# aelefebv/nellie

Hardware: AMD Instinct MI355X
Metric: Mvoxel/s multiscale Frangi (5 sigma) + Label, float32, frame resident in HBM (higher is better)
Workload: dtype f32; 1 GPU; synthetic 1024x1024x1024 float32 volume (N(100,5) noise + Gaussian tube segments, seed 2345), 0.1 um isotropic, 5-scale Frangi + Label, full hot path per step, frame resident in HBM; voxels=1073741824, labels=265, one_pass_scales=5, fast_div_proven=2, hessian_tile_rows=16

## Files before the change

### include/nellie_amd.h

```cpp
#ifndef NELLIE_AMD_H
#define NELLIE_AMD_H

#include <stddef.h>
#include <stdint.h>

#ifdef __cplusplus
extern "C" {
#endif

#define NL_OK      0
#define NL_EINVAL  1
#define NL_ENODEV  2
#define NL_ENOMEM  3
#define NL_EHIP    4
#define NL_ESTATE  5
#define NL_ECOMM   6

#define NL_U8 0
#define NL_I8 1
#define NL_U16 2
#define NL_I16 3
#define NL_U32 4
#define NL_I32 5
#define NL_F32 6
// ... 4 lines not shown
#define NL_FIELD_GAUSS  0
#define NL_FIELD_FROB   1
#define NL_FIELD_FRANGI 2
#define NL_FIELD_VESSELNESS 3

typedef struct nl_ctx nl_ctx;

const char *nl_version(void);

int nl_device_count(int *count, char *err, size_t errlen);
int nl_device_mem_info(int device, int64_t *free_bytes, int64_t *total_bytes, char *err, size_t errlen);
int nl_device_name(int device, char *name, size_t namelen, char *err, size_t errlen);

int nl_ctx_create(nl_ctx **out, int device,
                  int64_t nz_local, int64_t ny, int64_t nx,
                  int64_t gz0, int64_t gnz, int64_t own_lo, int64_t own_hi,
                  char *err, size_t errlen);
int nl_ctx_destroy(nl_ctx *ctx);
int nl_sync(nl_ctx *ctx, char *err, size_t errlen);
int64_t nl_ctx_bytes(int64_t nz_local, int64_t ny, int64_t nx);


int nl_filter_load(nl_ctx *ctx, const void *host, int dtype, int64_t z0, int64_t z1,
                   char *err, size_t errlen);

int nl_input_load(nl_ctx *ctx, const void *host, int dtype, int64_t z0, int64_t z1,
                  char *err, size_t errlen);
int nl_filter_begin(nl_ctx *ctx, char *err, size_t errlen);

int nl_gauss_step(nl_ctx *ctx,
                  const double *wz, int rz, const double *wy, int ry, const double *wx, int rx,
                  int64_t z0, int64_t z1, char *err, size_t errlen);

int nl_gauss_step_ahead(nl_ctx *ctx, const double *wz, int rz, const double *wy, int ry, const double *wx, int rx,
                        int64_t z0, int64_t z1, char *err, size_t errlen);
int nl_gauss_commit(nl_ctx *ctx, char *err, size_t errlen);

int nl_sample_gather(nl_ctx *ctx, int field, int64_t sz, int64_t sy, int64_t sx,
                     float *out, int64_t cap, int64_t *n, char *err, size_t errlen);

int nl_sample_gather_positive(nl_ctx *ctx, int field, int64_t sz, int64_t sy, int64_t sx,
                              float *out, int64_t cap, int64_t *n, char *err, size_t errlen);
int nl_sample_gather_positive_begin(nl_ctx *ctx, int field, int64_t sz, int64_t sy, int64_t sx, int64_t *n_lattice, char *err, size_t errlen);
int nl_sample_gather_positive_end(nl_ctx *ctx, float *out, int64_t cap, int64_t *n, char *err, size_t errlen);

int nl_sample_minmax(nl_ctx *ctx, int field, int64_t sz, int64_t sy, int64_t sx,
                     float *mn, float *mx, int64_t *npos, char *err, size_t errlen);

int nl_sample_hist(nl_ctx *ctx, int field, int64_t sz, int64_t sy, int64_t sx,
                   const float *edges, int nbins, int64_t *counts, char *err, size_t errlen);

int nl_sample_range_hist(nl_ctx *ctx, int field, int64_t sz, int64_t sy, int64_t sx, int nbins, float *mn, float *mx,
                         int64_t *n_positive, int64_t *counts, float *edges, int *valid, char *err, size_t errlen);
int nl_sample_range_hist2(nl_ctx *ctx, int field_a, int field_b, int64_t sz, int64_t sy, int64_t sx, int nbins, float *mn, float *mx,
                          int64_t *npos, int64_t *counts, float *edges, int *valid, char *err, size_t errlen);

int nl_hist_thresholds(const int64_t *counts, const float *edges, int nbins, double *triangle, double *otsu, int *status,
                       char *err, size_t errlen);
int nl_hist_thresholds_ex(const int64_t *counts, const void *edges, int edges_f64, int nbins, double *triangle, double *otsu,
                          double *otsu_var, int *status, char *err, size_t errlen);
int nl_host_hist_thresholds_f32(const float *values, int64_t n, int nbins, double *triangle, double *otsu, int *status,
                                int64_t *counts_out, float *edges_out, char *err, size_t errlen);

int nl_hessian_stats(nl_ctx *ctx, const double spacing[3],
                     float *max_abs, float *max_frob_sq, int *any_inf, char *err, size_t errlen);

int nl_set_frob_norm(nl_ctx *ctx, float max_abs, float max_finite, char *err, size_t errlen);

int nl_vesselness_step(nl_ctx *ctx, float gamma_sq, float alpha_sq, float beta_sq,
                       int use_thr, float thr, int64_t z0, int64_t z1, int64_t *mask_count,
                       char *err, size_t errlen);

int nl_set_spacing(nl_ctx *ctx, const double spacing[3], char *err, size_t errlen);

int nl_vesselness_spec(nl_ctx *ctx, const double spacing[3], float fsq_lo, float fsq_hi, int64_t z0, int64_t z1,
                       float *max_abs, float *max_frob_sq, int *any_inf, int *overflow, char *err, size_t errlen);

int nl_chain_begin(nl_ctx *ctx, int n_scales, char *err, size_t errlen);
int nl_chain_scale(nl_ctx *ctx, const double spacing[3], int64_t sz, int64_t sy, int64_t sx, double alpha_sq, double beta_sq,
                   double division, double margin, double test_scale, int64_t z0, int64_t z1, char *err, size_t errlen);
int nl_chain_flush(nl_ctx *ctx, char *err, size_t errlen);
int nl_chain_finish(nl_ctx *ctx, int *flags, double *gamma, double *max_abs, double *thr, int64_t *mask_count, char *err, size_t errlen);
int nl_chain_log(nl_ctx *ctx, int k, int which, int64_t *counts, float *edges, float *range, double *scalars, char *err, size_t errlen);

int nl_vesselness_resolve(nl_ctx *ctx, float gamma_sq, float alpha_sq, float beta_sq, int use_thr, float thr,
                          int *hit, int64_t *mask_count, char *err, size_t errlen);

int nl_vesselness_count(nl_ctx *ctx, int64_t *mask_count, char *err, size_t errlen);

int nl_set_ndim(nl_ctx *ctx, int ndim, char *err, size_t errlen);

int nl_log2d_step(nl_ctx *ctx, const double *wy2, const double *wy0, const double *wx2, const double *wx0, int r,
                  float s2, int first, int use_mask, char *err, size_t errlen);

int nl_log2d_finish(nl_ctx *ctx, int64_t *n_positive, char *err, size_t errlen);

int nl_filter_finish(nl_ctx *ctx, int64_t z0, int64_t z1, int64_t *n_positive, char *err, size_t errlen);

int nl_remove_edges(nl_ctx *ctx, int margin, int64_t *n_positive, char *err, size_t errlen);

int nl_mask_volume(nl_ctx *ctx, float thr, char *err, size_t errlen);

int nl_mask_volume_fused(nl_ctx *ctx, float thr, int64_t *n_positive, char *err, size_t errlen);
int nl_tail_enqueue(nl_ctx *ctx, int64_t sz, int64_t sy, int64_t sx, double q, char *err, size_t errlen);
int nl_tail_finish(nl_ctx *ctx, int commit, int64_t *n_samples, float *a, float *b, float *gamma, float *thr, int64_t *n_positive,
                   char *err, size_t errlen);
int nl_mask_volume_dev(nl_ctx *ctx, int64_t sz, int64_t sy, int64_t sx, double q, int64_t *n_samples, float *a, float *b, float *gamma,
                       float *thr, char *err, size_t errlen);
int nl_debug_percentile(nl_ctx *ctx, const float *values, int64_t n, double q, float *thr, float *a, float *b, char *err, size_t errlen);

int nl_filter_store(nl_ctx *ctx, float *host, int64_t z0, int64_t z1, char *err, size_t errlen);

int nl_gauss_store(nl_ctx *ctx, float *host, int64_t z0, int64_t z1, char *err, size_t errlen);


int nl_planes_get(nl_ctx *ctx, int field, int64_t z0, int64_t z1, float *host, char *err, size_t errlen);
int nl_planes_put(nl_ctx *ctx, int field, int64_t z0, int64_t z1, const float *host, char *err, size_t errlen);

int nl_comm_unique_id(char *id128, char *err, size_t errlen);
int nl_comm_init(nl_ctx *ctx, int world, int rank, const char *id128, char *err, size_t errlen);
int nl_comm_loopback_id(char *id128, char *err, size_t errlen);

int nl_halo_exchange(nl_ctx *ctx, int field, int64_t depth, char *err, size_t errlen);
int nl_halo_exchange_at(nl_ctx *ctx, int field, int64_t offset, int64_t depth, int async, char *err, size_t errlen);
int nl_comm_init2(nl_ctx *ctx, int world, int rank, const char *id128, char *err, size_t errlen);

int nl_allreduce(nl_ctx *ctx, void *host_inout, int64_t count, int dtype, int op, char *err, size_t errlen);


int nl_label_load_frangi(nl_ctx *ctx, const float *host, int64_t z0, int64_t z1,
                         char *err, size_t errlen);

int nl_label_intensity_mask(nl_ctx *ctx, const void *host_original, int dtype, double thresh,
                            char *err, size_t errlen);
int nl_label_intensity_mask_planes(nl_ctx *ctx, const void *host_original, int dtype, double thresh, int64_t z0, int64_t z1,
                                   char *err, size_t errlen);
int nl_label_intensity_mask_int(nl_ctx *ctx, const void *host_original, int dtype, int64_t thresh, int64_t z0, int64_t z1,
                                char *err, size_t errlen);

int nl_flat_sample_gather(nl_ctx *ctx, int field, int64_t offset, int64_t step,
                          float *out, int64_t cap, int64_t *n, char *err, size_t errlen);

int nl_flat_sample_gather_positive(nl_ctx *ctx, int field, int64_t offset, int64_t step, float *out, int64_t cap,
                                   int64_t *n, char *err, size_t errlen);

int nl_label_run(nl_ctx *ctx, int has_thr, float thr, int64_t min_area, int fill_holes,
                 int64_t *n_labels, char *err, size_t errlen);

int nl_label_pack(nl_ctx *ctx, int has_thr, float thr, char *err, size_t errlen);
int nl_label_bits_get(nl_ctx *ctx, int64_t row0, int64_t nrows, uint64_t *host, char *err, size_t errlen);
int nl_label_bits_put(nl_ctx *ctx, int64_t row0, int64_t nrows, const uint64_t *host, char *err, size_t errlen);
int nl_label_bits_allgather(nl_ctx *ctx, const int64_t *slab_plane0, char *err, size_t errlen);
int nl_label_run_global(nl_ctx *ctx, int64_t min_area, int fill_holes, int64_t *n_labels, char *err, size_t errlen);

int nl_slab_label_pack(nl_ctx *ctx, int has_thr, float thr, char *err, size_t errlen);
int nl_slab_bits_get(nl_ctx *ctx, int which, int64_t plane, uint64_t *host, char *err, size_t errlen);
int nl_slab_bits_put(nl_ctx *ctx, int which, int64_t plane, const uint64_t *host, char *err, size_t errlen);
int nl_slab_bits_exchange(nl_ctx *ctx, int which, char *err, size_t errlen);
int nl_slab_phase(nl_ctx *ctx, int phase, int gather, int64_t block_ints, int32_t *out, int64_t *need_ints, int64_t *nruns,
                  char *err, size_t errlen);
int nl_slab_patch(nl_ctx *ctx, int64_t n, const int32_t *roots, const int32_t *values, char *err, size_t errlen);
int nl_slab_apply(nl_ctx *ctx, int64_t min_area, char *err, size_t errlen);
int nl_slab_majority(nl_ctx *ctx, char *err, size_t errlen);
int nl_slab_number(nl_ctx *ctx, int64_t n_clear, const int32_t *clear, int64_t n_set, const int32_t *set, int64_t *n_local,
                   int32_t *ids_of_set, char *err, size_t errlen);
int nl_slab_paint(nl_ctx *ctx, int64_t base, int64_t n, const int32_t *roots, const int32_t *labels, char *err, size_t errlen);
// ... 152 lines not shown
```

### nellie_amd/csrc/chain.inc

```
#define NL_CHAIN_BINS 256
#define NL_CHAIN_MAX_SCALES 16

struct ChainHist {
    unsigned long long counts[NL_CHAIN_BINS];
    float edges[NL_CHAIN_BINS + 1];
    float pad_[3];
    unsigned int res[8];
};
static_assert(sizeof(ChainHist) == hist_layout(NL_CHAIN_BINS).bytes && offsetof(ChainHist, edges) == hist_layout(NL_CHAIN_BINS).off_edges &&
              offsetof(ChainHist, res) == hist_layout(NL_CHAIN_BINS).off_res, "ChainHist is hist_layout");

enum {
    NL_CF_GAUSS_HIST = 1, NL_CF_RAW_HIST = 2, NL_CF_TRIANGLE = 4, NL_CF_BRACKET = 8, NL_CF_INF = 16, NL_CF_OVERFLOW = 32,
    NL_CF_NORM_RANGE = 64, NL_CF_MISS = 128, NL_CF_EMPTY = 256, NL_CF_VERIFY = 512
};

struct ChainScale {
    float fsq_lo, fsq_hi;
    float gamma_sq, fsq_min;
    int m_inf, flags;
    float norm[2];
    unsigned int stats[4];
    unsigned long long cnt_walk, cnt_resolve;
    float gamma, max_abs, max_frob, thr, thr_cmp, raw_mn, raw_mx, nmn, nmx;
    int status_gauss, status_raw, status_exact;
    double tri[3], otsu[3];
    ChainHist h_gauss, h_raw, h_exact;
};

__device__ inline int wave_argmax_f64(const double *a, int n) {
    const int lane = threadIdx.x & 63;
    double best = 0.0; int at = 0x7fffffff; int first_nan = 0x7fffffff;
    for (int i = lane; i < n; i += 64) {
        const double v = a[i];
        if (v != v) { if (i < first_nan) first_nan = i; }
        else if (at == 0x7fffffff || v > best) { best = v; at = i; }
    }
#pragma unroll
    for (int o = 32; o > 0; o >>= 1) {
        const int onan = __shfl_xor(first_nan, o, 64);
        first_nan = onan < first_nan ? onan : first_nan;
        const double ob = __shfl_xor(best, o, 64);
        const int oa = __shfl_xor(at, o, 64);
        if (oa != 0x7fffffff && (at == 0x7fffffff || ob > best || (ob == best && oa < at))) { best = ob; at = oa; }
    }
    return first_nan != 0x7fffffff ? first_nan : (at == 0x7fffffff ? 0 : at);
}

__device__ inline void dev_hist_thresholds(const unsigned long long *counts, const float *edges, int nbins, double *scratch,
                                           double *triangle, double *otsu, int *status) {
    const int lane = threadIdx.x & 63;
    double *p = scratch, *pc = scratch + nbins, *w1 = scratch + 2 * nbins, *a1 = scratch + 3 * nbins, *w2 = scratch + 4 * nbins,
           *a2 = scratch + 5 * nbins;
    unsigned long long part = 0;
    for (int i = lane; i < nbins; i += 64) part += counts[i];
    const long long total = (long long)wave_sum_u64(part);
    for (int i = lane; i < nbins; i += 64) {
        const float centre = (edges[i] + edges[i + 1]) / 2.0f;
        const double pi = (double)(long long)counts[i] / (double)total;
        p[i] = pi;
        pc[i] = pi * (double)centre;
    }
    __syncthreads();
    if (nbins == 4 * 64) {
        double pv[4], qv[4], o1[4], o2[4];
#pragma unroll
        for (int j = 0; j < 4; ++j) { pv[j] = p[4 * lane + j]; qv[j] = pc[4 * lane + j]; }
        auto bcast = [](double v, int src) -> double {
            const unsigned long long b = (unsigned long long)__double_as_longlong(v);
            const unsigned int lo = (unsigned int)__builtin_amdgcn_readlane((int)(unsigned int)b, src);
            const unsigned int hi = (unsigned int)__builtin_amdgcn_readlane((int)(unsigned int)(b >> 32), src);
            return __longlong_as_double((long long)(((unsigned long long)hi << 32) | lo));
        };
        double acc = 0.0, accm = 0.0;
        for (int src = 0; src < 64; ++src) {
            double a = acc, m = accm;
            if (lane == src) {
#pragma unroll
                for (int j = 0; j < 4; ++j) { a += pv[j]; m += qv[j]; o1[j] = a; o2[j] = m; }
            }
            acc = bcast(a, src); accm = bcast(m, src);
        }
#pragma unroll
        for (int j = 0; j < 4; ++j) { w1[4 * lane + j] = o1[j]; a1[4 * lane + j] = o2[j]; }
        acc = 0.0; accm = 0.0;
        for (int src = 63; src >= 0; --src) {
            double a = acc, m = accm;
            if (lane == src) {
#pragma unroll
                for (int j = 3; j >= 0; --j) { a += pv[j]; m += qv[j]; o1[j] = a; o2[j] = m; }
            }
            acc = bcast(a, src); accm = bcast(m, src);
        }
#pragma unroll
        for (int j = 0; j < 4; ++j) { w2[4 * lane + j] = o1[j]; a2[4 * lane + j] = o2[j]; }
    } else if (lane == 0) {
        double acc = 0.0, accm = 0.0;
        for (int i = 0; i < nbins; ++i) { acc += p[i]; accm += pc[i]; w1[i] = acc; a1[i] = accm; }
        acc = 0.0; accm = 0.0;
        for (int i = nbins - 1; i >= 0; --i) { acc += p[i]; accm += pc[i]; w2[i] = acc; a2[i] = accm; }
    }
    __syncthreads();
    if (nbins < 2) *otsu = (double)((edges[0] + edges[1]) / 2.0f);
    else {
        double *var = pc;
        for (int i = lane; i + 1 < nbins; i += 64) {
            const double m1 = a1[i] / w1[i], m2 = a2[i + 1] / w2[i + 1];
            const double d = m1 - m2;
            var[i] = (w1[i] * w2[i + 1]) * (d * d);
        }
        __syncthreads();
        const int at = wave_argmax_f64(var, nbins - 1);
        *otsu = (double)((edges[at] + edges[at + 1]) / 2.0f);
    }
    __syncthreads();
    *status = 0;
    int peak = wave_argmax_f64(p, nbins);
    const double height = p[peak];
    int lo = 0x7fffffff, hi = -1;
    for (int i = lane; i < nbins; i += 64)
        if (p[i] != 0.0) { if (i < lo) lo = i; if (i > hi) hi = i; }
#pragma unroll
    for (int o = 32; o > 0; o >>= 1) {
        const int ol = __shfl_xor(lo, o, 64), oh = __shfl_xor(hi, o, 64);
        lo = ol < lo ? ol : lo; hi = oh > hi ? oh : hi;
    }
    if (lo == 0x7fffffff) lo = -1;
    const bool mirrored = (peak - lo) < (hi - peak);
    if (mirrored) { lo = nbins - hi - 1; peak = nbins - peak - 1; }
    const int span = peak - lo;
    if (span <= 0 || lo < 0) { *status = 1; *triangle = 0.0; return; }
    const double norm = sqrt(height * height + (double)((long long)span * (long long)span));
    const double hn = height / norm, sn = (double)span / norm;
    double *dist = w1;
    __syncthreads();
    for (int k = lane; k < span; k += 64) {
        const int bin = mirrored ? nbins - 1 - (k + lo) : k + lo;
        dist[k] = hn * (double)k - sn * p[bin];
    }
    __syncthreads();
    int level = wave_argmax_f64(dist, span) + lo;
    if (mirrored) level = nbins - level - 1;
    *triangle = (double)((edges[level] + edges[level + 1]) / 2.0f);
}

__device__ inline bool dev_finite_f(float x) { return fabsf(x) <= 3.402823466e38f; }

__global__ void __launch_bounds__(64)
chain_thr1_kernel(ChainScale *cs, double division, double margin, double test_scale) {
    __shared__ double scratch[6 * NL_CHAIN_BINS];
    int flags = 0;
    if (blockIdx.x == 0) {
        float gamma = 1.1920929e-07f;
        double tri0 = 0.0, otsu0 = 0.0;
        int st0 = 0;
        const ChainHist &h = cs->h_gauss;
        const unsigned long long cnt = *(const unsigned long long *)(h.res + 2);
        if (cnt == 0ull || h.res[4] != 1u) flags |= NL_CF_GAUSS_HIST;
        else {
            dev_hist_thresholds(h.counts, h.edges, NL_CHAIN_BINS, scratch, &tri0, &otsu0, &st0);
            if (st0) flags |= NL_CF_TRIANGLE;
            const float g = fminf((float)tri0, (float)otsu0);
            if (g > 0.0f) gamma = g;
        }
        const double g64 = (double)gamma;
        const float gamma_sq = (float)(2.0 * (g64 * g64));
        if (threadIdx.x == 0) {
            cs->gamma = gamma; cs->gamma_sq = gamma_sq;
            cs->tri[0] = tri0; cs->otsu[0] = otsu0; cs->status_gauss = st0;
            if (flags) atomicOr(&cs->flags, flags);
        }
        return;
    }
    float lo = __int_as_float(0x7f800000), hi = __int_as_float(0x7f800000);
    double tri1 = 0.0, otsu1 = 0.0;
    int st1 = 0;
    const ChainHist &h = cs->h_raw;
    const float raw_mn = __uint_as_float(h.res[0]), raw_mx = __uint_as_float(h.res[1]);
    const unsigned long long cnt = *(const unsigned long long *)(h.res + 2);
    if (cnt == 0ull || h.res[4] != 1u || !dev_finite_f(raw_mx)) flags |= NL_CF_RAW_HIST;
    else {
        dev_hist_thresholds(h.counts, h.edges, NL_CHAIN_BINS, scratch, &tri1, &otsu1, &st1);
        if (st1) flags |= NL_CF_TRIANGLE;
        const float tf = fminf((float)tri1, (float)otsu1);
        const double t = (double)tf * test_scale / division;
        const float l = (float)(t * t * (1.0 - margin)), u = (float)(t * t * (1.0 + margin));
        if (!(dev_finite_f(l) && dev_finite_f(u) && u > 0.0f) || !(l <= u)) flags |= NL_CF_BRACKET;
        else { lo = l; hi = u; }
    }
    if (threadIdx.x == 0) {
        cs->tri[1] = tri1; cs->otsu[1] = otsu1; cs->status_raw = st1;
        cs->raw_mn = raw_mn; cs->raw_mx = raw_mx;
        cs->fsq_lo = lo; cs->fsq_hi = hi;
        if (flags) atomicOr(&cs->flags, flags);
    }
}

__global__ void __launch_bounds__(64)
chain_post_kernel(ChainScale *cs) {
    if (threadIdx.x != 0) return;
    int flags = 0;
    const float max_abs32 = __uint_as_float(cs->stats[0]), max_fsq32 = __uint_as_float(cs->stats[1]);
    if (cs->stats[2]) flags |= NL_CF_INF;
    if (cs->stats[3]) flags |= NL_CF_OVERFLOW;
    const float max_abs = (max_abs32 <= 0.0f) ? 1.0f : max_abs32;
    cs->max_abs = max_abs;
    cs->max_frob = sqrtf(max_fsq32) / max_abs;
    cs->norm[0] = max_abs; cs->norm[1] = 0.0f;
    const float mn = cs->raw_mn / max_abs, mx = cs->raw_mx / max_abs;
    cs->nmn = mn; cs->nmx = mx;
    unsigned int *res = cs->h_exact.res;
    res[0] = __float_as_uint(mn); res[1] = __float_as_uint(mx); res[2] = 1u; res[3] = 0u; res[4] = 0u;
    if (!(mn > 0.0f && dev_finite_f(mx)) || (cs->flags & NL_CF_RAW_HIST)) { flags |= NL_CF_NORM_RANGE; res[2] = 0u; }
    cs->flags |= flags;
}

__device__ inline float dev_mask_threshold_on_fsq(float max_abs, float thr) {
    auto pred = [&](float x) -> bool { float fr = sqrtf(x); fr = fr / max_abs; return fr > thr; };
    unsigned int lo = 0u, hi = 0x7f7fffffu;
    if (!pred(__uint_as_float(hi))) return __int_as_float(0x7f800000);
    while (lo < hi) {
        const unsigned int mid = lo + (hi - lo) / 2;
        if (pred(__uint_as_float(mid))) hi = mid; else lo = mid + 1;
    }
    return __uint_as_float(lo);
}

__global__ void __launch_bounds__(64)
chain_thr2_kernel(ChainScale *cs, double division) {
    __shared__ double scratch[6 * NL_CHAIN_BINS];
    int flags = 0, st = 0, m_inf = 0;
    double tri = 0.0, otsu = 0.0;
    float thr = 0.0f, thr_cmp = 0.0f, fsq_min = __int_as_float(0x7f800000);
    const ChainHist &h = cs->h_exact;
    if (h.res[4] != 1u || (cs->flags & NL_CF_NORM_RANGE)) flags |= NL_CF_NORM_RANGE;
    else {
        dev_hist_thresholds(h.counts, h.edges, NL_CHAIN_BINS, scratch, &tri, &otsu, &st);
        if (st) flags |= NL_CF_TRIANGLE;
        thr = fminf((float)tri, (float)otsu);
        thr_cmp = (float)((double)thr / division);
        if (!(cs->max_frob > thr_cmp)) flags |= NL_CF_EMPTY;
        fsq_min = dev_mask_threshold_on_fsq(cs->max_abs, thr_cmp);
        m_inf = (0.0f > thr_cmp) ? 1 : 0;
        if (!(fsq_min >= cs->fsq_lo && fsq_min <= cs->fsq_hi)) flags |= NL_CF_MISS;
    }
    if (threadIdx.x == 0) {
        cs->tri[2] = tri; cs->otsu[2] = otsu; cs->status_exact = st;
        cs->thr = thr; cs->thr_cmp = thr_cmp; cs->fsq_min = fsq_min; cs->m_inf = m_inf;
        cs->flags |= flags;
    }
}

__global__ void __launch_bounds__(256)
chain_init_kernel(ChainScale *cs, int n) {
    const size_t words = sizeof(ChainScale) / 4 * (size_t)n;
    unsigned int *w = (unsigned int *)cs;
    for (size_t i = (size_t)blockIdx.x * blockDim.x + threadIdx.x; i < words; i += (size_t)gridDim.x * blockDim.x) w[i] = 0u;
    __syncthreads();
}
__global__ void __launch_bounds__(64)
chain_init2_kernel(ChainScale *cs, int n) {
    const int k = threadIdx.x;
    if (k < n) { cs[k].h_gauss.res[0] = 0xffffffffu; cs[k].h_raw.res[0] = 0xffffffffu; }
}
```

### nellie_amd/csrc/nellie_hip.hip

```cpp
#include "nl_host.h"

#include "hessian.inc"
#include "hessian_pair.inc"
#include "hv_launch.h"
#include "filter2d.inc"
#include "thresholds.inc"
#include "chain.inc"
#include "percentile.inc"


bool gyx_tiled() {
    static int on = -1;
    if (on < 0) { const char *e = getenv("NELLIE_GYX_TILE"); on = (e && !atoi(e)) ? 0 : 1; }
    return on != 0;
}
static unsigned resolve_grid(unsigned blocks) {
    static long cap = -1;
    if (cap < 0) { const char *e = getenv("NELLIE_RESOLVE_GRID"); cap = e ? atol(e) : 8192; }
    return (cap > 0 && (unsigned)cap < blocks) ? (unsigned)cap : blocks;
}
static int hm_ty() {
    static int v = -1;
    if (v < 0) { const char *e = getenv("NELLIE_HM_TY"); v = (e && atoi(e) == 16) ? 16 : 8; }
    return v;
// ... 66 lines not shown
    if (e != hipSuccess) {
        *count = 0;
        return nl_fail(err, errlen, NL_ENODEV, "hipGetDeviceCount: %s", hipGetErrorString(e));
    }
    *count = n;
    return NL_OK;
}

extern "C" int nl_device_mem_info(int device, int64_t *free_bytes, int64_t *total_bytes, char *err, size_t errlen) {
    NL_HIP(hipSetDevice(device));
    size_t f = 0, t = 0;
    NL_HIP(hipMemGetInfo(&f, &t));
    if (free_bytes) *free_bytes = (int64_t)f;
    if (total_bytes) *total_bytes = (int64_t)t;
    return NL_OK;
}

extern "C" int nl_device_name(int device, char *name, size_t namelen, char *err, size_t errlen) {
    hipDeviceProp_t p;
    NL_HIP(hipGetDeviceProperties(&p, device));
    if (name && namelen) snprintf(name, namelen, "%s (%s, %d CUs)", p.name, p.gcnArchName, p.multiProcessorCount);
    return NL_OK;
}

static int64_t vq_padded_plane(int64_t ny, int64_t nx) { return ((nx + HM_TX - 1) / HM_TX) * HM_TX * (((ny + 31) / 32) * 32); }
static int64_t vq_chunks(int64_t nzl, int64_t ny, int64_t nx) {
    static int64_t lim = 0;
    if (!lim) { const char *e = getenv("NELLIE_VQ_CAP"); lim = (e && atoll(e) > 0) ? atoll(e) : ((int64_t)1 << 28); }
    const int64_t per_chunk = vq_padded_plane(ny, nx) * HM_ZCHUNK;
    int64_t chunks = lim / per_chunk;
    const int64_t need = (nzl + HM_ZCHUNK - 1) / HM_ZCHUNK;
    if (chunks > need) chunks = need;
    return chunks < 1 ? 1 : chunks;
}
static int64_t vq_entries(int64_t nzl, int64_t ny, int64_t nx) { return vq_chunks(nzl, ny, nx) * vq_padded_plane(ny, nx) * HM_ZCHUNK; }
static int64_t vq_spec_regions(int64_t nzl, int64_t ny, int64_t nx) {
    return vq_padded_plane(ny, nx) / 64 * ((nzl + HM_ZCHUNK - 1) / HM_ZCHUNK);
}
static int64_t vq_spec_entries(int64_t nzl, int64_t ny, int64_t nx) {
    static int64_t lim = -1;
    if (lim < 0) { const char *e = getenv("NELLIE_SPEC_MAX_GB"); lim = (e ? atoll(e) : 64) << 30; }
    const int64_t ent = vq_spec_regions(nzl, ny, nx) * HM_SPEC_CAP;
    return ent * 32 <= lim ? ent : 0;
}
int64_t vq_alloc_entries(int64_t nzl, int64_t ny, int64_t nx) {
    const int64_t a = vq_entries(nzl, ny, nx), b = vq_spec_entries(nzl, ny, nx);
    return a > b ? a : b;
}
static int64_t vq_alloc_regions(int64_t nzl, int64_t ny, int64_t nx) {
    const int64_t a = vq_entries(nzl, ny, nx) / HM_REGION, b = vq_spec_entries(nzl, ny, nx) ? vq_spec_regions(nzl, ny, nx) : 0;
    return a > b ? a : b;
}

extern "C" int64_t nl_ctx_bytes(int64_t nz_local, int64_t ny, int64_t nx) {
    const int64_t n = nz_local * ny * nx;
    const int64_t qe = vq_alloc_entries(nz_local, ny, nx);
    return n * (4 * 4 + 3) + qe * 32 + vq_alloc_regions(nz_local, ny, nx) * 4 + (1 << 16) + ((n + SCAN_CHUNK - 1) / SCAN_CHUNK + 1) * 4;
}

extern "C" int nl_ctx_destroy(nl_ctx *c) {
    if (!c) return NL_OK;
    hipSetDevice(c->device);
    if (c->stream) hipStreamSynchronize(c->stream);
    for (auto &kv : c->prof) for (auto &r : kv.second) { hipEventDestroy(r.a); hipEventDestroy(r.b); }
    for (auto &r : c->prof_pool) { hipEventDestroy(r.a); hipEventDestroy(r.b); }
    for (int k = 0; k < 4; ++k) if (c->f[k]) hipFree(c->f[k]);
    for (int k = 0; k < 3; ++k) if (c->m[k]) hipFree(c->m[k]);
    if (c->d_small) hipFree(c->d_small);
    if (c->d_input && !c->input_borrowed) hipFree(c->d_input);
    for (int k = 0; k < 2; ++k) { if (c->d_in_slot[k]) hipFree(c->d_in_slot[k]); if (c->ev_in[k]) hipEventDestroy(c->ev_in[k]); }
    if (c->d_stage_fr) hipFree(c->d_stage_fr);
    if (c->d_stage_lab) hipFree(c->d_stage_lab);
    if (c->ev_staged) hipEventDestroy(c->ev_staged);
    if (c->ev_fetched) hipEventDestroy(c->ev_fetched);
    if (c->side) { hipStreamSynchronize(c->side); hipStreamDestroy(c->side); }
    if (c->ev_side) hipEventDestroy(c->ev_side);
    if (c->ev_main) hipEventDestroy(c->ev_main);
    if (c->ev_ahead) hipEventDestroy(c->ev_ahead);
    if (c->copy_in) hipStreamDestroy(c->copy_in);
    if (c->copy_out) hipStreamDestroy(c->copy_out);
    if (c->d_blk) hipFree(c->d_blk);
    for (int k = 0; k < 4; ++k) if (c->d_2d[k]) hipFree(c->d_2d[k]);
    if (c->d_fsq_cache) hipFree(c->d_fsq_cache);
    if (c->d_vq) hipFree(c->d_vq);
    if (c->mk_scratch) hipFree(c->mk_scratch);
    if (c->mk_act) hipFree(c->mk_act);
    if (c->d_vq_count) hipFree(c->d_vq_count);
    if (c->d_rows) hipFree(c->d_rows);
    if (c->d_ag) hipFree(c->d_ag);
    if (c->d_sl) hipFree(c->d_sl);
    if (c->d_seg_done) hipFree(c->d_seg_done);
    nw_release(c);
    if (c->d_pct) hipFree(c->d_pct);
    if (c->h_pct) hipHostFree(c->h_pct);
    if (c->h_sl) hipHostFree(c->h_sl);
    if (c->d_pack) hipFree(c->d_pack);
    if (c->h_ag) hipHostFree(c->h_ag);
    if (c->gbits[0]) hipFree(c->gbits[0]);
    if (c->gbits[1]) hipFree(c->gbits[1]);
    if (c->grows) hipFree(c->grows);
    if (c->h_small) hipHostFree(c->h_small);
    if (c->h_prefix) hipHostFree(c->h_prefix);
    if (c->t0) hipEventDestroy(c->t0);
    if (c->t1) hipEventDestroy(c->t1);
    if (c->xstream) { hipStreamSynchronize(c->xstream); hipStreamDestroy(c->xstream); }
    if (c->ev_x_main) hipEventDestroy(c->ev_x_main);
    if (c->ev_x_done) hipEventDestroy(c->ev_x_done);
    if (c->d_chain) hipFree(c->d_chain);
    if (c->h_chain) hipHostFree(c->h_chain);
    if (c->ev_chain) hipEventDestroy(c->ev_chain);
    comm_release(c, c->comm2, 2);
    comm_release(c, c->comm, 1);
    if (c->stream) hipStreamDestroy(c->stream);
    delete c;
    return NL_OK;
}

extern "C" int nl_ctx_create(nl_ctx **out, int device, int64_t nzl, int64_t ny, int64_t nx,
                             int64_t gz0, int64_t gnz, int64_t own_lo, int64_t own_hi, char *err, size_t errlen) {
    if (!out) return nl_fail(err, errlen, NL_EINVAL, "out is NULL");
    *out = nullptr;
    if (nzl < 1 || ny < 1 || nx < 1) return nl_fail(err, errlen, NL_EINVAL, "empty volume (%lld,%lld,%lld)", (i64)nzl, (i64)ny, (i64)nx);
    if (gz0 < 0 || gz0 + nzl > gnz) return nl_fail(err, errlen, NL_EINVAL, "slab [%lld,%lld) outside the global volume of %lld planes", (i64)gz0, (i64)(gz0 + nzl), (i64)gnz);
    if (own_lo < 0 || own_hi > nzl || own_lo >= own_hi) return nl_fail(err, errlen, NL_EINVAL, "bad owned range [%lld,%lld)", (i64)own_lo, (i64)own_hi);
    const i64 n = (i64)nzl * ny * nx;
    if (n >= ((i64)1 << 31)) return nl_fail(err, errlen, NL_EINVAL, "local slab of %lld voxels exceeds the int32 label index range; shard over Z", n);
    if (ny > 65535 || nzl > 65535) return nl_fail(err, errlen, NL_EINVAL, "Y and local Z extents must be <= 65535");
    int ndev = 0;
    hipError_t e = hipGetDeviceCount(&ndev);
    if (e != hipSuccess || ndev <= 0)
        return nl_fail(err, errlen, NL_ENODEV, "GPU backend requested but no HIP device is available (%s)", e == hipSuccess ? "0 devices" : hipGetErrorString(e));
    if (device < 0 || device >= ndev) return nl_fail(err, errlen, NL_ENODEV, "GPU backend requested but device %d does not exist (%d devices)", device, ndev);
    NL_HIP(hipSetDevice(device));
    nl_ctx *c = new nl_ctx();
    c->device = device; c->nzl = nzl; c->ny = ny; c->nx = nx; c->gz0 = gz0; c->gnz = gnz;
    c->own_lo = own_lo; c->own_hi = own_hi; c->n = n;
    int rc = NL_OK;
    auto alloc = [&](void **p, size_t bytes) -> bool {
        hipError_t ee = hipMalloc(p, bytes);
        if (ee != hipSuccess) {
            rc = nl_fail(err, errlen, ee == hipErrorOutOfMemory ? NL_ENOMEM : NL_EHIP,
                         "hipMalloc(%zu bytes): %s%s", bytes, hipGetErrorString(ee), ee == hipErrorOutOfMemory ? " [out of memory]" : "");
            return false;
        }
        return true;
    };
    bool ok = true;
    for (int k = 0; k < 4 && ok; ++k) ok = alloc((void **)&c->f[k], (size_t)n * 4);
    const size_t mask_words = (size_t)NL_MASK_SLOTS * nzl * ny * ((nx + 63) / 64);
    const size_t plane_words_bytes = (size_t)nzl * ny * ((nx + 63) / 64) * 8;
    for (int k = 0; k < 3 && ok; ++k) {
        size_t bytes = (size_t)n;
        if (k == 0 && mask_words * 8 > bytes) bytes = mask_words * 8;
        if (plane_words_bytes > bytes) bytes = plane_words_bytes;
        ok = alloc((void **)&c->m[k], bytes);
    }
    if (ok) ok = alloc((void **)&c->d_rows, ((size_t)nzl * ny + 2) * 2 * 4);
    if (ok) ok = alloc(&c->d_small, 1 << 16);
    c->vq_chunks = (int)vq_chunks(nzl, ny, nx);
    {
        const size_t qe = (size_t)vq_alloc_entries(nzl, ny, nx);
        if (ok) ok = alloc((void **)&c->d_vq, qe * 32);
        if (ok) ok = alloc((void **)&c->d_vq_count, (size_t)vq_alloc_regions(nzl, ny, nx) * 4);
        c->spec_ok = vq_spec_entries(nzl, ny, nx) > 0;
    }
    c->blk_cap = (n + SCAN_CHUNK - 1) / SCAN_CHUNK + 1;
    if (ok) ok = alloc(&c->d_blk, (size_t)c->blk_cap * 4);
    if (ok && hipHostMalloc(&c->h_small, 1 << 16, hipHostMallocDefault) != hipSuccess) {
        rc = nl_fail(err, errlen, NL_ENOMEM, "hipHostMalloc failed [out of memory]"); ok = false;
    }
    int side_prio = -1;
    { const char *e = getenv("NELLIE_SIDE_PRIO"); if (e) side_prio = atoi(e); }
    int prio_lo = 0, prio_hi = 0;
    (void)hipDeviceGetStreamPriorityRange(&prio_lo, &prio_hi);
    const int side_p = side_prio < 0 ? prio_hi : (side_prio > 0 ? prio_lo : (prio_lo + prio_hi) / 2);
    if (ok && (hipStreamCreateWithPriority(&c->side, hipStreamNonBlocking, side_p) != hipSuccess ||
               hipEventCreateWithFlags(&c->ev_side, hipEventDisableTiming) != hipSuccess ||
               hipEventCreateWithFlags(&c->ev_main, hipEventDisableTiming) != hipSuccess ||
               hipEventCreateWithFlags(&c->ev_ahead, hipEventDisableTiming) != hipSuccess)) {
        rc = nl_fail(err, errlen, NL_EHIP, "stream/event creation failed"); ok = false;
    }
    if (ok && (hipStreamCreateWithFlags(&c->stream, hipStreamNonBlocking) != hipSuccess ||
               hipEventCreate(&c->t0) != hipSuccess || hipEventCreate(&c->t1) != hipSuccess)) {
        rc = nl_fail(err, errlen, NL_EHIP, "stream/event creation failed"); ok = false;
    }
    if (!ok) { nl_ctx_destroy(c); return rc; }
    *out = c;
    return NL_OK;
}

extern "C" int nl_sync(nl_ctx *c, char *err, size_t errlen) {
    if (!c) return nl_fail(err, errlen, NL_EINVAL, "ctx is NULL");
    NL_HIP(hipSetDevice(c->device));
    NL_HIP(hipStreamSynchronize(c->stream));
    NL_HIP(hipStreamSynchronize(c->side));
    if (c->xstream) NL_HIP(hipStreamSynchronize(c->xstream));
    return NL_OK;
}


int upload_convert(nl_ctx *c, const void *host, int dtype, float *dst, i64 count, char *err, size_t errlen) {
    const size_t es = dtype_size(dtype);
    if (!es) return nl_fail(err, errlen, NL_EINVAL, "unsupported dtype code %d", dtype);
    if (dtype == NL_F32) {
        NL_HIP(hipMemcpyAsync(dst, host, (size_t)count * 4, hipMemcpyHostToDevice, c->stream));
        NL_HIP(hipStreamSynchronize(c->stream));
        return NL_OK;
    }
    void *raw = nullptr;
    bool own = false;
    for (int k = 0; k < 4 && !raw; ++k) {
        const bool contains = (dst >= c->f[k] && dst < c->f[k] + c->n);
        if (!contains && k != c->i_vmax && es <= 4) raw = c->f[k];
    }
    if (!raw) { NL_HIP(hipMalloc(&raw, (size_t)count * es)); own = true; }
    NL_HIP(hipMemcpyAsync(raw, host, (size_t)count * es, hipMemcpyHostToDevice, c->stream));
    const unsigned int g = grid1d(count);
    switch (dtype) {
        case NL_U8: convert_kernel<uint8_t><<<g, 256, 0, c->stream>>>((const uint8_t *)raw, dst, count); break;
        case NL_I8: convert_kernel<int8_t><<<g, 256, 0, c->stream>>>((const int8_t *)raw, dst, count); break;
        case NL_U16: convert_kernel<uint16_t><<<g, 256, 0, c->stream>>>((const uint16_t *)raw, dst, count); break;
        case NL_I16: convert_kernel<int16_t><<<g, 256, 0, c->stream>>>((const int16_t *)raw, dst, count); break;
        case NL_U32: convert_kernel<uint32_t><<<g, 256, 0, c->stream>>>((const uint32_t *)raw, dst, count); break;
        case NL_I32: convert_kernel<int32_t><<<g, 256, 0, c->stream>>>((const int32_t *)raw, dst, count); break;
        case NL_F64: convert_kernel<double><<<g, 256, 0, c->stream>>>((const double *)raw, dst, count); break;
        case NL_U64: convert_kernel<uint64_t><<<g, 256, 0, c->stream>>>((const uint64_t *)raw, dst, count); break;
        case NL_I64: convert_kernel<int64_t><<<g, 256, 0, c->stream>>>((const int64_t *)raw, dst, count); break;
    }
    NL_CHECK_LAUNCH();
    NL_HIP(hipStreamSynchronize(c->stream));
    if (own) hipFree(raw);
    return NL_OK;
}

extern "C" int nl_filter_load(nl_ctx *c, const void *host, int dtype, int64_t z0, int64_t z1, char *err, size_t errlen) {
    NL_ENTER(c);
    NL_JOIN_SIDE(c);
    if (!host || z0 < 0 || z1 > c->nzl || z0 >= z1) return nl_fail(err, errlen, NL_EINVAL, "bad plane range [%lld,%lld)", (i64)z0, (i64)z1);
    c->i_gauss = 0; c->i_vmax = 3; c->i_labels = -1; c->frangi_ready = 0;
    c->pz_on = 0; c->prezero_used = 0;
    c->gauss_ext = nullptr;
    if (c->ahead_pending) NL_HIP(hipStreamWaitEvent(c->stream, c->ev_ahead, 0));
    c->ahead_pending = 0;
    c->fsq_cache_valid = 0;
    NL_HIP(zero_small((char *)c->d_small + (52 << 10), 4, c->stream));
    c->vmax_zero_lo = c->vmax_zero_hi = 0;
    const i64 plane = c->ny * c->nx;
    int rc = upload_convert(c, host, dtype, c->f[0] + z0 * plane, (z1 - z0) * plane, err, errlen);
    if (rc) return rc;
    c->mask_slots_used = 0;
    NL_HIP(hipStreamSynchronize(c->stream));
    return NL_OK;
}

extern "C" int nl_input_load(nl_ctx *c, const void *host, int dtype, int64_t z0, int64_t z1, char *err, size_t errlen) {
    NL_ENTER(c);
    const size_t es = dtype_size(dtype);
    if (!es) return nl_fail(err, errlen, NL_EINVAL, "unsupported dtype code %d", dtype);
    if (!host || z0 < 0 || z1 > c->nzl || z0 >= z1) return nl_fail(err, errlen, NL_EINVAL, "bad plane range [%lld,%lld)", (i64)z0, (i64)z1);
    if (c->d_input && c->input_borrowed) { c->d_input = nullptr; c->input_borrowed = 0; }
    if (c->d_input && c->input_dtype != dtype) { hipFree(c->d_input); c->d_input = nullptr; }
    if (!c->d_input) NL_HIP(hipMalloc(&c->d_input, (size_t)c->n * es));
    c->input_dtype = dtype;
    const i64 plane = c->ny * c->nx;
    NL_HIP(hipMemcpyAsync((char *)c->d_input + (size_t)z0 * plane * es, host, (size_t)(z1 - z0) * plane * es, hipMemcpyHostToDevice, c->stream));
    NL_HIP(hipStreamSynchronize(c->stream));
    return NL_OK;
}

extern "C" int nl_filter_begin(nl_ctx *c, char *err, size_t errlen) {
    NL_ENTER(c);
    NL_JOIN_SIDE(c);
    if (!c->d_input) return nl_fail(err, errlen, NL_ESTATE, "nl_filter_begin before nl_input_load");
    c->i_gauss = 0; c->i_vmax = 3; c->i_labels = -1; c->frangi_ready = 0;
    c->pz_on = 0; c->prezero_used = 0;
    c->mask_slots_used = 0;
    c->gauss_ext = nullptr;
    if (c->ahead_pending) NL_HIP(hipStreamWaitEvent(c->stream, c->ev_ahead, 0));
    c->ahead_pending = 0;
    c->fsq_cache_valid = 0;
    NL_HIP(zero_small((char *)c->d_small + (52 << 10), 4, c->stream));
    c->vmax_zero_lo = c->vmax_zero_hi = 0;
    if (c->input_dtype == NL_F32 && !getenv("NELLIE_COPY_INPUT")) {
        c->gauss_ext = (float *)c->d_input;
        return NL_OK;
    }
    ProfScope ps(c, "load");
    const unsigned int g = grid1d(c->n);
    switch (c->input_dtype) {
        case NL_U8: convert_kernel<uint8_t><<<g, 256, 0, c->stream>>>((const uint8_t *)c->d_input, c->f[0], c->n); break;
        case NL_I8: convert_kernel<int8_t><<<g, 256, 0, c->stream>>>((const int8_t *)c->d_input, c->f[0], c->n); break;
        case NL_U16: convert_kernel<uint16_t><<<g, 256, 0, c->stream>>>((const uint16_t *)c->d_input, c->f[0], c->n); break;
        case NL_I16: convert_kernel<int16_t><<<g, 256, 0, c->stream>>>((const int16_t *)c->d_input, c->f[0], c->n); break;
        case NL_U32: convert_kernel<uint32_t><<<g, 256, 0, c->stream>>>((const uint32_t *)c->d_input, c->f[0], c->n); break;
        case NL_I32: convert_kernel<int32_t><<<g, 256, 0, c->stream>>>((const int32_t *)c->d_input, c->f[0], c->n); break;
        case NL_F32: convert_kernel<float><<<g, 256, 0, c->stream>>>((const float *)c->d_input, c->f[0], c->n); break;
        case NL_F64: convert_kernel<double><<<g, 256, 0, c->stream>>>((const double *)c->d_input, c->f[0], c->n); break;
        case NL_U64: convert_kernel<uint64_t><<<g, 256, 0, c->stream>>>((const uint64_t *)c->d_input, c->f[0], c->n); break;
        case NL_I64: convert_kernel<int64_t><<<g, 256, 0, c->stream>>>((const int64_t *)c->d_input, c->f[0], c->n); break;
    }
    NL_CHECK_LAUNCH();
    c->mask_slots_used = 0;
    return NL_OK;
}


static bool gauss_can_yx(const nl_ctx *c, const double *wy, int ry, const double *wx, int rx) {
    return wy && wx && ry == rx && ry >= 1 && ry <= GM_MAX_R && ry <= c->ny && !getenv("NELLIE_NO_FUSED_YX");
}
static int gauss_step_volumes(const nl_ctx *c, const double *wz, const double *wy, int ry, const double *wx, int rx) {
    return (wz ? 1 : 0) + (gauss_can_yx(c, wy, ry, wx, rx) ? 1 : (wy ? 1 : 0) + (wx ? 1 : 0));
}

extern "C" int nl_gauss_step(nl_ctx *c, const double *wz, int rz, const double *wy, int ry, const double *wx, int rx,
                             int64_t z0, int64_t z1, char *err, size_t errlen) {
    NL_ENTER(c);
    if (c->ahead_pending) return nl_fail(err, errlen, NL_ESTATE, "nl_gauss_step while a step enqueued ahead is uncommitted");
    if (z0 < 0 || z1 > c->nzl || z0 >= z1) return nl_fail(err, errlen, NL_EINVAL, "bad plane range [%lld,%lld)", (i64)z0, (i64)z1);
    if (c->halo_pending) {
        ProfScope ps(c, "halo_wait");
        NL_HIP(hipStreamWaitEvent(c->stream, c->ev_x_done, 0));
        c->halo_pending = 0;
    }
    const VolGeom v = geom(c);
    const dim3 grid((unsigned)((c->nx + 255) / 256), (unsigned)c->ny, (unsigned)(z1 - z0));
    int src = c->i_gauss;
    const float *srcp = gauss_cur(c);
    GaussW gw;
    int rc;
    const bool can_yx = gauss_can_yx(c, wy, ry, wx, rx);
    bool fused_yx = false;
    const char *e_fz = getenv("NELLIE_GAUSS_FUSED");
    const bool fused_zyx = e_fz ? atoi(e_fz) != 0 : c->n >= ((i64)1 << 26);
    if (fused_zyx && wz && can_yx && gyx_tiled() && gl_zyx_ok(c, rz, ry, c->f[(src + 1) % 3]) &&
        memcmp(wy, wx, (size_t)(2 * ry + 1) * sizeof(double)) == 0) {
        GaussW gy;
        if ((rc = fill_gw(gw, wz, rz, err, errlen)) || (rc = fill_gw(gy, wy, ry, err, errlen))) return rc;
        if ((z0 - rz < 0 && c->gz0 > 0) || (z1 - 1 + rz >= c->nzl && c->gz0 + c->nzl < c->gnz))
            return nl_fail(err, errlen, NL_EINVAL, "Z pass of radius %d on planes [%lld,%lld) reaches outside the local slab", rz, (i64)z0, (i64)z1);
        const int dst = (src + 1) % 3;
        char scope[32];
        snprintf(scope, sizeof scope, "gauss_zyx<%d,%d>", rz, ry);
        ProfScope ps(c, scope);
        static int zero_in_passing = -1;
        if (zero_in_passing < 0) { const char *e = getenv("NELLIE_ZERO_IN_GAUSS"); zero_in_passing = (e && !atoi(e)) ? 0 : 1; }
        const bool zero = zero_in_passing && c->mask_slots_used == 0 && c->vmax_zero_hi == 0 && c->stream != c->side;
        const bool ahead = c->stream == c->side;
        const bool prezero = !zero && c->pz_on && c->chain_n > 0 && c->chain_k == c->chain_n - (ahead ? 2 : 1) && z0 == 0 && z1 == c->nzl;
        float *third = c->f[(src + 2) % 3];
        (void)gl_zyx(c, rz, ry, srcp, c->f[dst], v, z0, z1, gauss_ws_of(gw), gauss_ws_of(gy), zero ? c->f[c->i_vmax] : (prezero ? third : nullptr));
        if (zero) { c->vmax_zero_lo = z0; c->vmax_zero_hi = z1; }
        NL_CHECK_LAUNCH();
        if (prezero) pz_set(c, third);
        src = dst; srcp = c->f[dst];
        fused_yx = true;
        wz = nullptr;
    }
    if (wz) {
        if ((rc = fill_gw(gw, wz, rz, err, errlen))) return rc;
        if ((z0 - rz < 0 && c->gz0 > 0) || (z1 - 1 + rz >= c->nzl && c->gz0 + c->nzl < c->gnz))
            return nl_fail(err, errlen, NL_EINVAL, "Z pass of radius %d on planes [%lld,%lld) reaches outside the local slab", rz, (i64)z0, (i64)z1);
        const int dst = (src + 1) % 3;
        ProfScope ps(c, "gauss_z");
        if (!gl_fast(0, c, srcp, c->f[dst], v, z0, z1, gw)) gl_axis(0, false, c, grid, srcp, c->f[dst], v, z0, z1, gw);
        NL_CHECK_LAUNCH();
        src = dst; srcp = c->f[dst];
    }
    if (!fused_yx && can_yx) {
        GaussW gy, gx;
        if ((rc = fill_gw(gy, wy, ry, err, errlen))) return rc;
        if ((rc = fill_gw(gx, wx, rx, err, errlen))) return rc;
        const GaussWS wsy = gauss_ws_of(gy), wsx = gauss_ws_of(gx);
        const int dst = (src + 1) % 3;
        ProfScope ps(c, "gauss_yx");
        const dim3 g2((unsigned)((c->nx + GYX_COLS - 1) / GYX_COLS), (unsigned)((c->ny + v.chunk - 1) / v.chunk), (unsigned)(z1 - z0));
        (void)gl_yx(c, gyx_tiled(), false, ry, srcp, c->f[dst], v, z0, z1, wsy, wsx, g2);
        NL_CHECK_LAUNCH();
        src = dst; srcp = c->f[dst];
        fused_yx = true;
    }
    if (wy && !fused_yx) {
        if ((rc = fill_gw(gw, wy, ry, err, errlen))) return rc;
        const int dst = (src + 1) % 3;
        ProfScope ps(c, "gauss_y");
        if (!gl_fast(1, c, srcp, c->f[dst], v, z0, z1, gw)) gl_axis(1, false, c, grid, srcp, c->f[dst], v, z0, z1, gw);
        NL_CHECK_LAUNCH();
        src = dst; srcp = c->f[dst];
    }
    if (wx && !fused_yx) {
        if ((rc = fill_gw(gw, wx, rx, err, errlen))) return rc;
        const int dst = (src + 1) % 3;
        ProfScope ps(c, "gauss_x");
        if (!gl_fast(2, c, srcp, c->f[dst], v, z0, z1, gw)) gl_axis(2, false, c, grid, srcp, c->f[dst], v, z0, z1, gw);
        NL_CHECK_LAUNCH();
        src = dst; srcp = c->f[dst];
    }
    c->i_gauss = src;
    c->fsq_cache_valid = 0;
    if (srcp != c->gauss_ext) c->gauss_ext = nullptr;
    return NL_OK;
}

extern "C" int nl_gauss_step_ahead(nl_ctx *c, const double *wz, int rz, const double *wy, int ry, const double *wx, int rx,
                                   int64_t z0, int64_t z1, char *err, size_t errlen) {
    NL_ENTER(c);
    if (c->ahead_pending) return nl_fail(err, errlen, NL_ESTATE, "a step enqueued ahead is already pending");
    if (gauss_step_volumes(c, wz, wy, ry, wx, rx) > 2)
        return nl_fail(err, errlen, NL_ESTATE, "a cascade step of three passes (radii %d / %d / %d) cannot run ahead: it needs the current Gaussian's volume", rz, ry, rx);
    NL_HIP(hipEventRecord(c->ev_main, c->stream));
    hipStream_t ahead_stream = c->side;
    NL_HIP(hipStreamWaitEvent(ahead_stream, c->ev_main, 0));
    const int cur_idx = c->i_gauss;
    float *cur_ext = c->gauss_ext;
    hipStream_t main_stream = c->stream;
    c->stream = ahead_stream;
    const int rc = nl_gauss_step(c, wz, rz, wy, ry, wx, rx, z0, z1, err, errlen);
    c->stream = main_stream;
    if (rc) { c->i_gauss = cur_idx; c->gauss_ext = cur_ext; return rc; }
    c->ahead_gauss = c->i_gauss;
    c->i_gauss = cur_idx; c->gauss_ext = cur_ext;
    NL_HIP(hipEventRecord(c->ev_ahead, ahead_stream));
    c->ahead_pending = 1;
    return NL_OK;
}

extern "C" int nl_gauss_commit(nl_ctx *c, char *err, size_t errlen) {
    NL_ENTER_KEEP_PZ(c);
    if (!c->ahead_pending) return nl_fail(err, errlen, NL_ESTATE, "nl_gauss_commit without nl_gauss_step_ahead");
    NL_HIP(hipStreamWaitEvent(c->stream, c->ev_ahead, 0));
    c->i_gauss = c->ahead_gauss;
    c->gauss_ext = nullptr;
    c->ahead_pending = 0;
    c->fsq_cache_valid = 0;
    return NL_OK;
}

static int set_spacing(nl_ctx *c, const double spacing[3], char *err, size_t errlen) {
    if (!spacing) return nl_fail(err, errlen, NL_EINVAL, "spacing is NULL");
    if ((!c->two_d && c->gnz < 2) || c->ny < 2 || c->nx < 2)
        return nl_fail(err, errlen, NL_EINVAL, "Shape of array too small to calculate a numerical gradient, at least (edge_order + 1) elements are required.");
    if (c->chk_spacing[0] != spacing[0] || c->chk_spacing[1] != spacing[1] || c->chk_spacing[2] != spacing[2]) c->fsq_cache_valid = 0;
    c->hz = (float)spacing[0]; c->hy = (float)spacing[1]; c->hx = (float)spacing[2];
    c->hz2 = (float)(2.0 * spacing[0]); c->hy2 = (float)(2.0 * spacing[1]); c->hx2 = (float)(2.0 * spacing[2]);
    if (!c->have_spacing || c->chk_spacing[0] != spacing[0] || c->chk_spacing[1] != spacing[1] || c->chk_spacing[2] != spacing[2]) {
        int rcx = check_fast_div(c, err, errlen);
        if (rcx) return rcx;
        c->chk_spacing[0] = spacing[0]; c->chk_spacing[1] = spacing[1]; c->chk_spacing[2] = spacing[2];
    }
    c->have_spacing = 1;
    return NL_OK;
}

extern "C" int nl_set_spacing(nl_ctx *c, const double spacing[3], char *err, size_t errlen) {
    NL_ENTER(c);
    return set_spacing(c, spacing, err, errlen);
}

extern "C" int nl_hessian_stats(nl_ctx *c, const double spacing[3], float *max_abs, float *max_frob_sq, int *any_inf,
                                char *err, size_t errlen) {
    NL_ENTER(c);
    { int rcs = set_spacing(c, spacing, err, errlen); if (rcs) return rcs; }
    c->spec_valid = 0;
    if (c->two_d) {
        unsigned int *res2 = (unsigned int *)c->d_small;
        NL_HIP(zero_small(res2, 16, c->stream));
        {
            ProfScope ps(c, "hessian_stats");
            hessian2d_stats_kernel<<<grid2d_rows(c->nx, c->ny), 256, 0, c->stream>>>(gauss_cur(c), geom(c), hessp(c), res2);
            NL_CHECK_LAUNCH();
        }
        unsigned int *h2 = (unsigned int *)c->h_small;
        NL_HIP(hipMemcpyAsync(h2, res2, 16, hipMemcpyDeviceToHost, c->stream));
        NL_HIP(hipStreamSynchronize(c->stream));
        if (max_abs) memcpy(max_abs, &h2[0], 4);
        if (max_frob_sq) memcpy(max_frob_sq, &h2[1], 4);
        if (any_inf) *any_inf = (int)h2[2];
        return NL_OK;
    }
    unsigned int *res = (unsigned int *)c->d_small;
    NL_HIP(zero_small(res, 16, c->stream));
    {
        ProfScope ps(c, "hessian_stats");
// ... 243 lines not shown
    *hit = 0;
    if (!c->spec_valid) return NL_OK;
    VessP vp = make_vessp(c, gamma_sq, alpha_sq, beta_sq, use_thr, thr);
    if (!(vp.fsq_min >= c->spec_lo && vp.fsq_min <= c->spec_hi)) { c->spec_valid = 0; return NL_OK; }
    unsigned long long *d_cnt = (unsigned long long *)((char *)c->d_small + (48 << 10));
    if (resolve_on_side()) {
        NL_HIP(hipEventRecord(c->ev_main, c->stream));
        NL_HIP(hipStreamWaitEvent(c->side, c->ev_main, 0));
        NL_HIP(zero_small(d_cnt, 8, c->side));
    } else {
        NL_HIP(zero_small(d_cnt, 8, c->stream));
    }
    { int rc = resolve_enqueue(c, vp, d_cnt, nullptr, err, errlen); if (rc) return rc; }
    *hit = 1;
    if (mask_count) {
        int rcc = nl_vesselness_count(c, mask_count, err, errlen);
        if (rcc) return rcc;
    }
    return NL_OK;
}


static inline unsigned int f2u(float x) { unsigned int u; memcpy(&u, &x, 4); return u; }
static inline float u2f(unsigned int u) { float x; memcpy(&x, &u, 4); return x; }
static inline float py_min_f(float a, float b) { return b < a ? b : a; }

static int chain_verify(const ChainScale &s, double division, double margin, double test_scale) {
    if (s.flags) return s.flags;
    int bad = 0;
    double tri, otsu; int st;
    {
        hist_thresholds_host<float>((const int64_t *)s.h_gauss.counts, s.h_gauss.edges, NL_CHAIN_BINS, &tri, &otsu, &st);
        const float g = py_min_f((float)tri, (float)otsu);
        const float gamma = g > 0.0f ? g : 1.1920929e-07f;
        const float gamma_sq = (float)(2.0 * std::pow((double)gamma, 2.0));
        if (st || f2u(gamma) != f2u(s.gamma) || f2u(gamma_sq) != f2u(s.gamma_sq)) bad = 1;
        float e[NL_CHAIN_BINS + 1];
        host_edges(u2f(s.h_gauss.res[0]), u2f(s.h_gauss.res[1]), NL_CHAIN_BINS, e);
        if (memcmp(e, s.h_gauss.edges, sizeof(e))) bad = 1;
    }
    {
        hist_thresholds_host<float>((const int64_t *)s.h_raw.counts, s.h_raw.edges, NL_CHAIN_BINS, &tri, &otsu, &st);
        const double t = (double)py_min_f((float)tri, (float)otsu) * test_scale / division;
        const float lo = (float)(t * t * (1.0 - margin)), hi = (float)(t * t * (1.0 + margin));
        if (st || f2u(lo) != f2u(s.fsq_lo) || f2u(hi) != f2u(s.fsq_hi)) bad = 1;
        float e[NL_CHAIN_BINS + 1];
        host_edges(u2f(s.h_raw.res[0]), u2f(s.h_raw.res[1]), NL_CHAIN_BINS, e);
        if (memcmp(e, s.h_raw.edges, sizeof(e))) bad = 1;
    }
    {
        const float max_abs32 = u2f(s.stats[0]), max_fsq32 = u2f(s.stats[1]);
        const float max_abs = max_abs32 <= 0.0f ? 1.0f : max_abs32;
        volatile float mf = sqrtf(max_fsq32); mf = mf / max_abs;
        volatile float mn = u2f(s.h_raw.res[0]) / max_abs, mx = u2f(s.h_raw.res[1]) / max_abs;
        if (f2u(max_abs) != f2u(s.max_abs) || f2u((float)mf) != f2u(s.max_frob) || f2u((float)mn) != f2u(s.nmn) || f2u((float)mx) != f2u(s.nmx) ||
            f2u(s.norm[0]) != f2u(max_abs) || s.norm[1] != 0.0f) bad = 1;
        float e[NL_CHAIN_BINS + 1];
        host_edges((float)mn, (float)mx, NL_CHAIN_BINS, e);
        if (memcmp(e, s.h_exact.edges, sizeof(e))) bad = 1;
        hist_thresholds_host<float>((const int64_t *)s.h_exact.counts, s.h_exact.edges, NL_CHAIN_BINS, &tri, &otsu, &st);
        const float thr = py_min_f((float)tri, (float)otsu);
        const float thr_cmp = (float)((double)thr / division);
        const float fsq_min = mask_threshold_on_fsq(max_abs, 1, thr_cmp);
        if (st || f2u(thr) != f2u(s.thr) || f2u(thr_cmp) != f2u(s.thr_cmp) || f2u(fsq_min) != f2u(s.fsq_min) || s.m_inf != ((0.0f > thr_cmp) ? 1 : 0)) bad = 1;
        if (!(fsq_min >= s.fsq_lo && fsq_min <= s.fsq_hi) || !((float)mf > thr_cmp)) bad = 1;
    }
    return bad ? NL_CF_VERIFY : 0;
}

extern "C" int nl_chain_begin(nl_ctx *c, int n_scales, char *err, size_t errlen) {
    NL_ENTER(c);
    if (n_scales < 1 || n_scales > NL_CHAIN_MAX_SCALES) return nl_fail(err, errlen, NL_EINVAL, "a chain holds 1..%d scales", NL_CHAIN_MAX_SCALES);
    if (!c->two_d && (!c->spec_ok || !hv_rs(c))) return nl_fail(err, errlen, NL_ESTATE, "the device-resident chain needs the 3-D one-pass walk");
    if (!c->d_chain) {
        NL_HIP(hipMalloc(&c->d_chain, sizeof(ChainScale) * NL_CHAIN_MAX_SCALES));
        NL_HIP(hipHostMalloc(&c->h_chain, sizeof(ChainScale) * NL_CHAIN_MAX_SCALES, hipHostMallocDefault));
        NL_HIP(hipEventCreateWithFlags(&c->ev_chain, hipEventDisableTiming));
    }
    chain_init_kernel<<<16, 256, 0, c->stream>>>((ChainScale *)c->d_chain, n_scales);
    chain_init2_kernel<<<1, 64, 0, c->stream>>>((ChainScale *)c->d_chain, n_scales);
    NL_CHECK_LAUNCH();
    c->chain_n = n_scales; c->chain_k = 0; c->chain_copy_pending = 0;
    c->def_resolve = 0;
    const char *e_pz = getenv("NELLIE_PREZERO");
    c->pz_on = (e_pz ? atoi(e_pz) != 0 : NL_PREZERO_DEFAULT) && !c->two_d && !c->comm && c->own_lo == 0 && c->own_hi == c->nzl && c->nzl == c->gnz;
    return NL_OK;
}

extern "C" int nl_chain_scale(nl_ctx *c, const double spacing[3], int64_t sz, int64_t sy, int64_t sx, double alpha_sq, double beta_sq,
                              double division, double margin, double test_scale, int64_t z0, int64_t z1, char *err, size_t errlen) {
    NL_ENTER_KEEP_PZ(c);
    if (!c->d_chain || c->chain_k >= c->chain_n) return nl_fail(err, errlen, NL_ESTATE, "nl_chain_scale outside nl_chain_begin .. nl_chain_finish");
    if (!(division != 0.0)) return nl_fail(err, errlen, NL_EINVAL, "the chain needs a non-zero threshold division");
    int rc;
    if ((rc = set_spacing(c, spacing, err, errlen))) return rc;
    if ((rc = resolve_deferred_launch(c, true, err, errlen))) return rc;
    ChainScale *cs = (ChainScale *)c->d_chain + c->chain_k;
    c->chain_par[c->chain_k][0] = division; c->chain_par[c->chain_k][1] = margin; c->chain_par[c->chain_k][2] = test_scale;
    ++c->chain_k;
    c->frob_max_abs = 1.0f; c->frob_max_finite = 0.0f;
    if (c->two_d) {
        if ((rc = sample_first_round(c, NL_FIELD_GAUSS, NL_FIELD_FROB, sz, sy, sx, NL_CHAIN_BINS, (char *)&cs->h_gauss, (char *)&cs->h_raw, nullptr, nullptr, true, err, errlen))) return rc;
        chain_thr1_kernel<<<2, 64, 0, c->stream>>>(cs, division, margin, test_scale);
        {
            ProfScope ps(c, "hessian_stats");
            hessian2d_stats_kernel<<<grid2d_rows(c->nx, c->ny), 256, 0, c->stream>>>(gauss_cur(c), geom(c), hessp(c), cs->stats);
        }
        chain_post_kernel<<<1, 64, 0, c->stream>>>(cs);
        NL_CHECK_LAUNCH();
        if ((rc = sample_exact_round(c, sz, sy, sx, NL_CHAIN_BINS, (char *)&cs->h_exact, cs->norm, c->stream, false, err, errlen))) return rc;
        chain_thr2_kernel<<<1, 64, 0, c->stream>>>(cs, division);
        NL_CHECK_LAUNCH();
        VessP vp{};
        vp.alpha_sq = (float)alpha_sq; vp.beta_sq = (float)beta_sq; vp.use_thr = 1;
        vp.cnt_lo = (int)c->own_lo; vp.cnt_hi = (int)c->own_hi;
        vp.first = c->mask_slots_used == 0 ? 1 : 0;
        vp.nan_flag = (unsigned int *)((char *)c->d_small + NL_NAN_FLAG_OFF);
        ProfScope ps(c, "vesselness");
        const int wpr = (int)((c->nx + 63) / 64);
        const i64 slot_words = c->nzl * c->ny * wpr;
        const int k_scale = c->mask_slots_used++;
        vp.have_prev = k_scale > 0;
        unsigned long long *cm = (unsigned long long *)c->m[0] + (i64)(k_scale & 1) * slot_words;
        const unsigned long long *pm = (unsigned long long *)c->m[0] + (i64)((k_scale + 1) & 1) * slot_words;
        if (vp.first && !vmax_is_zero(c, 0, c->nzl)) NL_HIP(hipMemsetAsync(c->f[c->i_vmax], 0, (size_t)c->n * 4, c->stream));
        c->vmax_zero_hi = 0;
        c->spec_valid = 0;
        vesselness2d_kernel<<<grid2d_rows((i64)wpr * 64, c->ny), 256, 0, c->stream>>>(gauss_cur(c), c->f[c->i_vmax], cm, pm, wpr, geom(c), hessp(c), vp,
                                                                                        &cs->cnt_resolve, (const float *)cs);
        NL_CHECK_LAUNCH();
        return NL_OK;
    }
    if ((rc = sample_first_round(c, NL_FIELD_GAUSS, NL_FIELD_FROB, sz, sy, sx, NL_CHAIN_BINS, (char *)&cs->h_gauss, (char *)&cs->h_raw, nullptr, nullptr, true, err, errlen))) return rc;
    chain_thr1_kernel<<<2, 64, 0, c->stream>>>(cs, division, margin, test_scale);
    NL_CHECK_LAUNCH();
    if ((rc = spec_enqueue(c, spacing, 0.0f, 0.0f, z0, z1, cs->stats, &cs->cnt_walk, &cs->fsq_lo, err, errlen))) return rc;
    const bool defer = resolve_defer_ok(c) && c->fsq_cache_valid;
    hipStream_t st = c->stream;
    chain_post_kernel<<<1, 64, 0, st>>>(cs);
    NL_CHECK_LAUNCH();
    if ((rc = sample_exact_round(c, sz, sy, sx, NL_CHAIN_BINS, (char *)&cs->h_exact, cs->norm, st, true, err, errlen))) return rc;
    chain_thr2_kernel<<<1, 64, 0, st>>>(cs, division);
    NL_CHECK_LAUNCH();
    VessP vp{};
    vp.alpha_sq = (float)alpha_sq; vp.beta_sq = (float)beta_sq; vp.use_thr = 1;
    vp.cnt_lo = (int)c->own_lo; vp.cnt_hi = (int)c->own_hi;
    vp.first = c->mask_slots_used == 0 ? 1 : 0;
    if (defer) {
        memcpy(c->def_vp, &vp, sizeof(VessP));
        c->def_cnt = &cs->cnt_resolve; c->def_params = (const float *)cs; c->def_resolve = 1;
        return NL_OK;
    }
    return resolve_enqueue(c, vp, &cs->cnt_resolve, (const float *)cs, err, errlen);
}

extern "C" int nl_chain_flush(nl_ctx *c, char *err, size_t errlen) {
    NL_ENTER_KEEP_PZ(c);
    if (!c->d_chain || c->chain_k < 1) return nl_fail(err, errlen, NL_ESTATE, "nl_chain_flush without scales");
    { int rcd = resolve_deferred_launch(c, false, err, errlen); if (rcd) return rcd; }
    NL_JOIN_SIDE(c);
    NL_HIP(hipMemcpyAsync(c->h_chain, c->d_chain, sizeof(ChainScale) * (size_t)c->chain_k, hipMemcpyDeviceToHost, c->stream));
    NL_HIP(hipEventRecord(c->ev_chain, c->stream));
    c->chain_copy_pending = 1;
    return NL_OK;
}

extern "C" int nl_chain_finish(nl_ctx *c, int *flags, double *gamma, double *max_abs, double *thr, int64_t *mask_count, char *err, size_t errlen) {
    NL_ENTER_KEEP_PZ(c);
    if (!c->d_chain || c->chain_k < 1) return nl_fail(err, errlen, NL_ESTATE, "nl_chain_finish without scales");
    const int n = c->chain_k;
    if (!c->chain_copy_pending) { int rcd = resolve_deferred_launch(c, false, err, errlen); if (rcd) return rcd; }
    if (c->chain_copy_pending) {
        NL_HIP(hipEventSynchronize(c->ev_chain));
        c->chain_copy_pending = 0;
    } else {
        NL_JOIN_SIDE(c);
        NL_HIP(hipMemcpyAsync(c->h_chain, c->d_chain, sizeof(ChainScale) * (size_t)n, hipMemcpyDeviceToHost, c->stream));
        NL_HIP(hipStreamSynchronize(c->stream));
    }
    const ChainScale *h = (const ChainScale *)c->h_chain;
    for (int k = 0; k < n; ++k) {
        const int f = chain_verify(h[k], c->chain_par[k][0], c->chain_par[k][1], c->chain_par[k][2]);
        if (flags) flags[k] = f;
        if (gamma) gamma[k] = (double)h[k].gamma;
        if (max_abs) max_abs[k] = (double)h[k].max_abs;
        if (thr) thr[k] = (double)h[k].thr;
        if (mask_count) mask_count[k] = (int64_t)(h[k].cnt_walk + h[k].cnt_resolve);
    }
    c->chain_n = 0; c->pz_on = 0;
    return NL_OK;
}

extern "C" int nl_chain_log(nl_ctx *c, int k, int which, int64_t *counts, float *edges, float *range, double *scalars, char *err, size_t errlen) {
    if (!c || !c->h_chain || k < 0 || k >= NL_CHAIN_MAX_SCALES || which < 0 || which > 2) return nl_fail(err, errlen, NL_EINVAL, "bad chain log request");
    const ChainScale &s = ((const ChainScale *)c->h_chain)[k];
    const ChainHist &h = which == 0 ? s.h_gauss : (which == 1 ? s.h_raw : s.h_exact);
    if (counts) memcpy(counts, h.counts, sizeof(h.counts));
    if (edges) memcpy(edges, h.edges, sizeof(h.edges));
    if (range) { range[0] = u2f(h.res[0]); range[1] = u2f(h.res[1]); }
    if (scalars) {
        scalars[0] = s.fsq_lo; scalars[1] = s.fsq_hi; scalars[2] = s.gamma_sq; scalars[3] = s.fsq_min; scalars[4] = s.thr_cmp; scalars[5] = s.max_frob;
        scalars[6] = s.tri[which]; scalars[7] = s.otsu[which];
    }
    return NL_OK;
}

extern "C" int nl_vesselness_step(nl_ctx *c, float gamma_sq, float alpha_sq, float beta_sq, int use_thr, float thr,
                                  int64_t z0, int64_t z1, int64_t *mask_count, char *err, size_t errlen) {
    NL_ENTER(c);
    if (z0 < 0 && z1 < 0) { z0 = c->own_lo; z1 = c->own_hi; }
    if (z0 < 0 || z1 > c->nzl || z0 >= z1) return nl_fail(err, errlen, NL_EINVAL, "bad plane range [%lld,%lld)", (i64)z0, (i64)z1);
    if (!c->have_spacing) return nl_fail(err, errlen, NL_ESTATE, "nl_vesselness_step before nl_hessian_stats");
    NL_JOIN_SIDE(c);
    unsigned long long *d_cnt = (unsigned long long *)c->d_small;
    NL_HIP(zero_small(d_cnt, 8, c->stream));
    VessP vp = make_vessp(c, gamma_sq, alpha_sq, beta_sq, use_thr, thr);
    vp.qcap = HM_REGION;
    c->spec_valid = 0;
    if (c->two_d) {
        ProfScope ps(c, "vesselness");
        const int wpr = (int)((c->nx + 63) / 64);
        const i64 slot_words = c->nzl * c->ny * wpr;
        const int k_scale = c->mask_slots_used++;
        vp.have_prev = k_scale > 0;
        unsigned long long *cm = (unsigned long long *)c->m[0] + (i64)(k_scale & 1) * slot_words;
        const unsigned long long *pm = (unsigned long long *)c->m[0] + (i64)((k_scale + 1) & 1) * slot_words;
        if (vp.first && !vmax_is_zero(c, 0, c->nzl)) NL_HIP(hipMemsetAsync(c->f[c->i_vmax], 0, (size_t)c->n * 4, c->stream));
        c->vmax_zero_hi = 0;
        vesselness2d_kernel<<<grid2d_rows((i64)wpr * 64, c->ny), 256, 0, c->stream>>>(gauss_cur(c), c->f[c->i_vmax], cm, pm, wpr, geom(c), hessp(c), vp, d_cnt);
        NL_CHECK_LAUNCH();
    } else {
        ProfScope ps(c, "vesselness");
        const int ntx = (int)((c->nx + HM_TX - 1) / HM_TX);
        const int wpr = (int)((c->nx + 63) / 64);
        const i64 slot_words = c->nzl * c->ny * wpr;
        const int k_scale = c->mask_slots_used++;
        vp.have_prev = k_scale > 0;
        unsigned long long *cm = (unsigned long long *)c->m[0] + (i64)(k_scale & 1) * slot_words;
        const unsigned long long *pm = (unsigned long long *)c->m[0] + (i64)((k_scale + 1) & 1) * slot_words;
        const i64 plane = c->ny * c->nx;
        const i64 planes_per_launch = (i64)c->vq_chunks * HM_ZCHUNK;
        const VQueue vq{(float4 *)c->d_vq, c->d_vq_count};
        if (vp.first && !vmax_is_zero(c, z0, z1))
            NL_HIP(hipMemsetAsync(c->f[c->i_vmax] + z0 * plane, 0, (size_t)(z1 - z0) * plane * 4, c->stream));
        c->vmax_zero_hi = 0;
        const int rs = hv_rs(c);
        const int ty = rs ? 2 * rs : hm_ty();
        const int nty = (int)((c->ny + ty - 1) / ty);
        if (rs) vp.qcap = 2 * hv_np(c) * HM_REGION;
#define NL_LAUNCH_VESS(TYV, FASTV, HR)                                                                                    \
        hessian_g_kernel<1, TYV, FASTV><<<nblocks, HGCfg<TYV>::NT, HGCfg<TYV>::lds_bytes(), c->stream>>>(                 \
            gauss_cur(c), cm, pm, wpr, geom(c), HR, vp, vq, (int)za, (int)zb, ntx, nty, nullptr, d_cnt)
        for (i64 za = z0; za < z1; za += planes_per_launch) {
            const i64 zb = za + planes_per_launch < z1 ? za + planes_per_launch : z1;
            const int nzc = (int)((zb - za + HM_ZCHUNK - 1) / HM_ZCHUNK);
            const unsigned nblocks = (unsigned)(ntx * nty * nzc);
            if (rs) NL_HIP(nl_hv_launch(HvLaunch{1, rs, hv_np(c), hv_fastv(c), nblocks, c->stream, gauss_cur(c), cm, pm, wpr, geom(c), hessp(c), vp, vq, (int)za, (int)zb,
                                                 ntx, nty, nullptr, d_cnt, nullptr}));
            else if (ty == 8) { if (c->fast_div) NL_LAUNCH_VESS(8, true, hessdv_fast(c)); else NL_LAUNCH_VESS(8, false, hessdv_exact(c)); }
            else { if (c->fast_div) NL_LAUNCH_VESS(16, true, hessdv_fast(c)); else NL_LAUNCH_VESS(16, false, hessdv_exact(c)); }
            NL_CHECK_LAUNCH();
            const unsigned nregions = nblocks * (unsigned)(rs ? rs / hv_np(c) : ty);
            vesselness_queue_kernel<false><<<resolve_grid((nregions + 3) / 4), 256, 0, c->stream>>>(vq.ent, vq.count, nregions, c->f[c->i_vmax], za * plane, vp,
                                                                                      nullptr, nullptr, wpr, (int)c->ny, (int)c->nx, za, nullptr, nullptr);
            NL_CHECK_LAUNCH();
        }
#undef NL_LAUNCH_VESS
        NL_CHECK_LAUNCH();
    }
    if (mask_count) {
        NL_HIP(hipMemcpyAsync(c->h_small, d_cnt, 8, hipMemcpyDeviceToHost, c->stream));
        NL_HIP(hipStreamSynchronize(c->stream));
// ... 474 lines not shown
```

### nellie_amd/csrc/nl_common.h

```cpp
#pragma once
#include <atomic>
#include <hip/hip_runtime.h>
#include <stdarg.h>
#include <stdint.h>
#include <stdio.h>
#include <string.h>
#include <string>
#include <vector>
#include <map>

#include "../../include/nellie_amd.h"

typedef long long i64;

struct ProfRec { hipEvent_t a, b; };

struct nl_ctx {
    int device = 0;
    hipStream_t stream = nullptr;
    i64 nzl = 0, ny = 0, nx = 0;
    i64 gz0 = 0, gnz = 0;
    i64 own_lo = 0, own_hi = 0;
    i64 n = 0;

// ... 31 lines not shown
    int *nw_feat = nullptr, *nw_stk = nullptr; i64 nw_scr_cap = 0;
    void *nw_objs = nullptr; i64 nw_objs_cap = 0;
    hipEvent_t nw_ev[2] = {nullptr, nullptr};
    float nw_ms[4] = {0, 0, 0, 0};
    int thin_valid = 0;
    i64 thin_counts[7] = {0, 0, 0, 0, 0, 0, 0};
    float thin_ms = 0;
    hipEvent_t thin_ev[2] = {nullptr, nullptr};
    const float *mk_int = nullptr;
    float *mk_use = nullptr;
    float *mk_scratch = nullptr;
    std::atomic<unsigned long long> epoch{0};
    unsigned long long support_epoch = ~0ull - 8;
    const unsigned long long *d_support = nullptr;
    unsigned long long labbits_epoch = ~0ull - 8;
    int last_label_sparse = 0;
    float *pz_buf = nullptr;
    unsigned long long pz_epoch = ~0ull - 8;
    int pz_on = 0;
    int prezero_used = 0;
    unsigned char *mk_act = nullptr; size_t mk_act_cap = 0;
    int mk_act_valid = 0;
    int mk_ntiles = 0;
    int mk_state = 0;
    int mk_first_scale = 1;
    int two_d = 0;
    float *d_2d[4] = {nullptr, nullptr, nullptr, nullptr};
    float *d_fsq_cache = nullptr;
    i64 fsq_cache_cap = 0, fsq_cache_key[3] = {0, 0, 0};
    int fsq_cache_valid = 0;
    float *gauss_ext = nullptr;
    int vq_chunks = 1;
    int spec_ok = 0;
    int spec_valid = 0;
    float spec_lo = 0, spec_hi = 0;
    i64 spec_z0 = 0, spec_z1 = 0;
    unsigned int spec_nregions = 0;
    int spec_qcap = 0;
    unsigned long long spec_count = 0;
    hipStream_t side = nullptr;
    hipEvent_t ev_side = nullptr, ev_main = nullptr;
    hipEvent_t ev_ahead = nullptr;
    int ahead_pending = 0, ahead_gauss = 0;
    int side_pending = 0;
    int def_resolve = 0;
    alignas(8) unsigned char def_vp[160] = {};
    unsigned long long *def_cnt = nullptr;
    const float *def_params = nullptr;
    int last_spec_overflow = 0;
    float last_fsq_min = 0;
    void *d_blk = nullptr;
    unsigned int *d_rows = nullptr;
    unsigned long long *gbits[2] = {nullptr, nullptr};
    unsigned int *grows = nullptr;
    int comm_poisoned = 0;
    i64 blk_cap = 0;
    i64 sl_e0 = 0, sl_e1 = 0;
    i64 sl_nruns = 0;
    int sl_phase = -1;
    int *d_sl = nullptr; size_t d_sl_ints = 0;
    int *h_sl = nullptr; size_t h_sl_ints = 0;
    int sl_capE = 0;
    int sl_numbered = 0;
    uint8_t *d_seg_done = nullptr; size_t seg_done_cap = 0;

    float hz = 1, hy = 1, hx = 1;
    float hz2 = 2, hy2 = 2, hx2 = 2;
    int have_spacing = 0;
    int fast_div = 0;
    int fast_div2 = 0;
    double chk_spacing[3] = {0, 0, 0};
    float frob_max_abs = 1.0f, frob_max_finite = 0.0f;
    int frangi_ready = 0;
    i64 vmax_zero_lo = 0, vmax_zero_hi = 0;
    int mask_slots_used = 0;
    hipEvent_t ev_chain = nullptr; int chain_copy_pending = 0;
    i64 gp_total = -1; float *gp_stage = nullptr;
    void *d_pct = nullptr;
    void *h_pct = nullptr;
    int tail_pending = 0, tail_dst = -1;
    void *d_chain = nullptr, *h_chain = nullptr;
    int chain_n = 0, chain_k = 0;
    double chain_par[16][3] = {};

    void *comm = nullptr;
    int fuse_reduce = 0;
    void *d_ag = nullptr; size_t ag_cap = 0;
    void *h_ag = nullptr; size_t h_ag_cap = 0;
    void *comm2 = nullptr;
    hipStream_t xstream = nullptr;
    hipEvent_t ev_x_main = nullptr, ev_x_done = nullptr;
    int halo_pending = 0;
    int world = 1, rank = 0;

    hipEvent_t t0 = nullptr, t1 = nullptr;
    int prof_on = 0;
    std::map<std::string, std::vector<ProfRec>> prof;
    std::map<std::string, std::pair<double, int64_t>> prof_sum;
    std::vector<ProfRec> prof_pool;
    std::vector<hipEvent_t> ev_pool;
};

static inline int nl_fail(char *err, size_t errlen, int code, const char *fmt, ...) {
    if (err && errlen) {
        va_list ap;
        va_start(ap, fmt);
        vsnprintf(err, errlen, fmt, ap);
        va_end(ap);
    }
    return code;
}

#define NL_HIP(expr)                                                                          \
    do {                                                                                      \
        hipError_t e_ = (expr);                                                               \
        if (e_ != hipSuccess) {                                                               \
            (void)hipGetLastError();    \
                                                   \
            int code_ = (e_ == hipErrorOutOfMemory) ? NL_ENOMEM                               \
                        : (e_ == hipErrorNoDevice || e_ == hipErrorInvalidDevice) ? NL_ENODEV \
                                                                                  : NL_EHIP;  \
            return nl_fail(err, errlen, code_, "%s: %s (%s:%d)%s", #expr, hipGetErrorString(e_), \
                           __FILE__, __LINE__, code_ == NL_ENOMEM ? " [out of memory]" : ""); \
        }                                                                                     \
    } while (0)

#define NL_CHECK_LAUNCH() NL_HIP(hipGetLastError())

static inline void prof_harvest(nl_ctx *c, bool all) {
    for (auto &kv : c->prof) {
        auto &v = kv.second;
        size_t k = 0;
        for (; k < v.size(); ++k) {
            if (!all && hipEventQuery(v[k].b) != hipSuccess) { (void)hipGetLastError(); break; }
            float t = 0;
            if (hipEventElapsedTime(&t, v[k].a, v[k].b) == hipSuccess) { auto &s = c->prof_sum[kv.first]; s.first += t; s.second += 1; }
            c->prof_pool.push_back(v[k]);
        }
        v.erase(v.begin(), v.begin() + k);
    }
}

struct ProfScope {
    nl_ctx *c; ProfRec r; bool on;
    hipStream_t st;
    ProfScope(nl_ctx *ctx, const char *name, hipStream_t stream = nullptr) : c(ctx), on(ctx->prof_on != 0), st(stream ? stream : ctx->stream) {
        if (!on) return;
        if (c->prof_pool.empty()) prof_harvest(c, false);
        if (!c->prof_pool.empty()) { r = c->prof_pool.back(); c->prof_pool.pop_back(); }
        else { hipEventCreate(&r.a); hipEventCreate(&r.b); }
        hipEventRecord(r.a, st);
        key = name;
    }
    ~ProfScope() { if (on) { hipEventRecord(r.b, st); c->prof[key].push_back(r); } }
    std::string key;
};
```

### nellie_amd/hipnative.py

```python
from __future__ import annotations

import ctypes as C
import os

import numpy as np

_HERE = os.path.dirname(os.path.abspath(__file__))
LIB_PATH = os.environ.get("NELLIE_HIP_LIB") or os.path.join(_HERE, "libnellie_hip.so")

NL_OK, NL_EINVAL, NL_ENODEV, NL_ENOMEM, NL_EHIP, NL_ESTATE, NL_ECOMM = range(7)
FIELD_GAUSS, FIELD_FROB, FIELD_FRANGI, FIELD_VESSELNESS = 0, 1, 2, 3

DTYPE_CODES = {
    np.dtype(np.uint8): 0, np.dtype(np.int8): 1, np.dtype(np.uint16): 2, np.dtype(np.int16): 3,
    np.dtype(np.uint32): 4, np.dtype(np.int32): 5, np.dtype(np.float32): 6, np.dtype(np.float64): 7,
    np.dtype(np.uint64): 8, np.dtype(np.int64): 9,
}

_ERRLEN = 512
_i64, _int, _f32, _f64 = C.c_int64, C.c_int, C.c_float, C.c_double
_p = C.c_void_p
_ERR = (C.c_char_p, C.c_size_t)

_PROTOS = {
# ... 27 lines not shown
    "nl_host_slab_join": [_int, _p, _i64, _i64, C.POINTER(_i64), C.POINTER(_i64), _p, _p, _p, _p],
    "nl_outputs_pack": [_p, _int, _p],
    "nl_outputs_pack_with_label": [_p, _int],
    "nl_outputs_fetch_packed_async": [_p, _p, _i64],
    "nl_outputs_unpack": [_p, _i64, _p, _p, _i64, _int, _int],
    "nl_host_zero": [_p, _i64, _int],
    "nl_hessian_stats": [_p, C.POINTER(_f64), C.POINTER(_f32), C.POINTER(_f32), C.POINTER(_int)],
    "nl_set_frob_norm": [_p, _f32, _f32],
    "nl_vesselness_step": [_p, _f32, _f32, _f32, _int, _f32, _i64, _i64, C.POINTER(_i64)],
    "nl_set_spacing": [_p, C.POINTER(_f64)],
    "nl_vesselness_spec": [_p, C.POINTER(_f64), _f32, _f32, _i64, _i64, C.POINTER(_f32), C.POINTER(_f32),
                           C.POINTER(_int), C.POINTER(_int)],
    "nl_vesselness_resolve": [_p, _f32, _f32, _f32, _int, _f32, C.POINTER(_int), C.POINTER(_i64)],
    "nl_vesselness_count": [_p, C.POINTER(_i64)],
    "nl_set_ndim": [_p, _int],
    "nl_markers_begin": [_p, _p, _p, _int],
    "nl_markers_distance": [_p, _f32, C.POINTER(_i64)],
    "nl_markers_log_step": [_p, C.POINTER(_f64), C.POINTER(_f64), _int, C.POINTER(_f64), C.POINTER(_f64), C.POINTER(_f64),
                            C.POINTER(_f64), _int, _f32],
    "nl_markers_finish": [_p, _int, C.POINTER(_i64)],
    "nl_markers_use_image": [_p, _p],
    "nl_markers_store": [_p, _p, _p, _p],
    "nl_skel_pixel_class": [_p, _p, _p, C.POINTER(_i64)],
    "nl_skel_branch_labels": [_p, _p, _p, C.POINTER(_i64)],
    "nl_network_load": [_p, _p, _p, _p, _int, C.POINTER(_i64)],
    "nl_network_clean_seed": [_p, C.POINTER(_i64), C.POINTER(_i64)],
    "nl_network_classes": [_p, C.POINTER(_i64), C.POINTER(_i64)],
    "nl_network_relabel_load": [_p, _p, _p, _int, C.POINTER(_i64)],
    "nl_network_relabel": [_p, C.POINTER(_f64), _i64, C.POINTER(_i64), C.POINTER(_i64), C.POINTER(_i64)],
    "nl_network_fetch": [_p, _p, _p, _p],
    "nl_network_kernel_ms": [_p, C.POINTER(_f32)],
    "nl_thin": [_p, _p, _p, _int, _int, C.POINTER(_i64)],
    "nl_network_load_thin": [_p, _p, _p, _int, _int, C.POINTER(_i64), C.POINTER(_i64)],
    "nl_network_fetch_mask": [_p, _p],
    "nl_thin_info": [_p, C.POINTER(_i64), C.POINTER(_f32)],
    "nl_mask_volume_fused": [_p, _f32, C.POINTER(_i64)],
    "nl_log2d_step": [_p, C.POINTER(_f64), C.POINTER(_f64), C.POINTER(_f64), C.POINTER(_f64), _int, _f32, _int, _int],
    "nl_log2d_finish": [_p, C.POINTER(_i64)],
    "nl_filter_finish": [_p, _i64, _i64, C.POINTER(_i64)],
    "nl_remove_edges": [_p, _int, C.POINTER(_i64)],
    "nl_planes_get": [_p, _int, _i64, _i64, _p],
    "nl_planes_put": [_p, _int, _i64, _i64, _p],
    "nl_comm_unique_id": [C.c_char_p],
    "nl_comm_loopback_id": [C.c_char_p],
    "nl_comm_init": [_p, _int, _int, C.c_char_p],
    "nl_halo_exchange": [_p, _int, _i64],
    "nl_halo_exchange_at": [_p, _int, _i64, _i64, _int],
    "nl_comm_init2": [_p, _int, _int, C.c_char_p],
    "nl_allreduce": [_p, _p, _i64, _int, _int],
    "nl_mask_volume": [_p, _f32],
    "nl_filter_store": [_p, _p, _i64, _i64],
    "nl_gauss_store": [_p, _p, _i64, _i64],
    "nl_label_load_frangi": [_p, _p, _i64, _i64],
    "nl_label_intensity_mask": [_p, _p, _int, _f64],
    "nl_label_intensity_mask_planes": [_p, _p, _int, _f64, _i64, _i64],
    "nl_label_intensity_mask_int": [_p, _p, _int, _i64, _i64, _i64],
    "nl_flat_sample_gather": [_p, _int, _i64, _i64, _p, _i64, C.POINTER(_i64)],
    "nl_flat_sample_gather_positive": [_p, _int, _i64, _i64, _p, _i64, C.POINTER(_i64)],
    "nl_label_run": [_p, _int, _f32, _i64, _int, C.POINTER(_i64)],
    "nl_label_store": [_p, _p, _i64, _i64],
    "nl_label_pack": [_p, _int, _f32],
    "nl_label_bits_get": [_p, _i64, _i64, _p],
    "nl_label_bits_put": [_p, _i64, _i64, _p],
    "nl_label_bits_allgather": [_p, _p],
    "nl_label_run_global": [_p, _i64, _int, C.POINTER(_i64)],
    "nl_slab_label_pack": [_p, _int, _f32],
    "nl_slab_bits_get": [_p, _int, _i64, _p],
    "nl_slab_bits_put": [_p, _int, _i64, _p],
    "nl_slab_bits_exchange": [_p, _int],
    "nl_slab_phase": [_p, _int, _int, _i64, _p, C.POINTER(_i64), C.POINTER(_i64)],
    "nl_slab_patch": [_p, _i64, _p, _p],
    "nl_slab_apply": [_p, _i64],
    "nl_slab_majority": [_p],
    "nl_slab_number": [_p, _i64, _p, _i64, _p, C.POINTER(_i64), _p],
    "nl_slab_paint": [_p, _i64, _i64, _p, _p],
    "nl_allgather_bytes": [_p, _p, _i64, _p, _i64, _p],
    "nl_allgather_var": [_p, _p, _i64, _p, _p, _p],
    "nl_comm_fuse": [_p, _int],
    "nl_chain_begin": [_p, _int],
    "nl_chain_scale": [_p, _p, _i64, _i64, _i64, _f64, _f64, _f64, _f64, _f64, _i64, _i64],
    "nl_chain_flush": [_p],
    "nl_chain_finish": [_p, _p, _p, _p, _p, _p],
    "nl_chain_log": [_p, _int, _int, _p, _p, _p, _p],
    "nl_pinned_alloc": [C.POINTER(_p), _i64],
    "nl_host_register": [_p, _i64],
    "nl_input_load_async": [_p, _int, _p, _int],
    "nl_input_select": [_p, _int],
    "nl_input_wait": [_p, _int],
    "nl_outputs_stage": [_p, _int],
    "nl_outputs_fetch_async": [_p, _p, _p],
    "nl_outputs_wait": [_p],
    "nl_debug_eig_frangi": [_p, _p, _i64, _int, _f32, _f32, _f32, _p],
    "nl_timer_begin": [_p],
    "nl_timer_end_ms": [_p, C.POINTER(_f32)],
    "nl_track_create": [C.POINTER(_p), _int, _int, _i64, _i64, _i64, _p],
    "nl_track_frame": [_p, _p, _int, _p, _p, _p, C.POINTER(_i64)],
    "nl_track_features": [_p, _int, _p, _p, _p],
    "nl_track_match": [_p, _int, _f64, _p, _p, _p, _p, _p],
    "nl_flow_create": [C.POINTER(_p), _int, _int, _p, _f64],
    "nl_flow_load": [_p, _p, _p, _p, _i64],
    "nl_flow_interpolate": [_p, _p, _i64, _p, C.POINTER(_i64)],
    "nl_flow_interpolate_dev": [_p, _p, _i64, _p, C.POINTER(_i64)],
    "nl_flow_kernel_ms": [_p, C.POINTER(_f32)],
    "nl_reassign_create": [C.POINTER(_p), _int, _int, _i64, _i64, _i64, _p, _f64],
    "nl_reassign_frame": [_p, _p, _p, _int, C.POINTER(_i64)],
    "nl_reassign_pair": [_p, _p, _p, C.POINTER(_i64)],
    "nl_reassign_fetch": [_p, _int, _p, _p, _p, _p],
    "nl_reassign_kernel_ms": [_p, C.POINTER(_f32)],
    "nl_voxfeat_create": [C.POINTER(_p), _int, _int, _i64, _i64, _i64, _p, _f64],
    "nl_voxfeat_frame": [_p, _p, _p, _p, _int, _p, _int, C.POINTER(_i64)],
    "nl_voxfeat_fetch_voxels": [_p, _p, _p, _p, _p, _p],
    "nl_voxfeat_motility": [_p, _p, _p, C.POINTER(_i64), C.POINTER(_i64)],
    "nl_voxfeat_fetch_motility": [_p, C.POINTER(_p)],
    "nl_voxfeat_nodes": [_p, _p, _int, _p, _int, C.POINTER(_i64), C.POINTER(_i64)],
    "nl_voxfeat_fetch_nodes": [_p, _p, _p, _p, _p, _p, _p, _p],
    "nl_voxfeat_kernel_ms": [_p, _p],
    "nl_nodefeat_create": [C.POINTER(_p), _int, _int, _i64, _i64, _i64, _p],
    "nl_nodefeat_frame": [_p, _p, _int, _p, _int, _p, _int, _p, _int, C.POINTER(_i64)],
    "nl_nodefeat_fetch": [_p, _p, _p, _p, _p],
    "nl_nodefeat_groups": [_p, _p, _p, _i64, C.POINTER(_i64)],
    "nl_nodefeat_set_wide_from": [_p, _i64],
    "nl_nodefeat_aggregate": [_p, _p, _int, _i64, _p],
    "nl_nodefeat_node_stats": [_p, _p, _p, _p, _i64, _p],
    "nl_nodefeat_kernel_ms": [_p, _p],
    "nl_branchfeat_create": [C.POINTER(_p), _int, _int, _i64, _i64, _i64, _p],
    "nl_branchfeat_frame": [_p, _p, _int, _p, _int, _p, _int, C.POINTER(_i64), C.POINTER(_i64), C.POINTER(_i64), C.POINTER(_i64)],
    "nl_branchfeat_fetch": [_p] * 12,
    "nl_branchfeat_regions": [_p, _p, _int, _p, _int, C.POINTER(_i64)],
    "nl_branchfeat_regions_rows": [_p, _p, _int, _p, _int, C.POINTER(_i64)],
    "nl_branchfeat_fetch_regions": [_p, _p, _p, _p],
    "nl_branchfeat_kernel_ms": [_p, _p],
    "nl_host_half_round": [_p, _p, _i64],
    "nl_host_half_nansum": [_p, _i64, _int, _p],
    "nl_host_np_sum_f32": [_p, _i64, _p],
}
_PLAIN = {
    "nl_version": (C.c_char_p, []),
    "nl_ctx_destroy": (_int, [_p]),
    "nl_ctx_bytes": (_i64, [_i64, _i64, _i64]),
    "nl_prof_enable": (_int, [_p, _int]),
    "nl_prof_get": (_int, [_p, C.c_char_p, C.POINTER(_f64), C.POINTER(_i64)]),
    "nl_prof_reset": (_int, [_p]),
    "nl_pinned_free": (_int, [_p]),
    "nl_host_unregister": (_int, [_p]),
    "nl_ctx_info": (_int, [_p, C.c_char_p, C.POINTER(_f64)]),
    "nl_track_destroy": (_int, [_p]),
    "nl_flow_destroy": (_int, [_p]),
    "nl_reassign_destroy": (_int, [_p]),
    "nl_voxfeat_destroy": (_int, [_p]),
    "nl_nodefeat_destroy": (_int, [_p]),
    "nl_branchfeat_destroy": (_int, [_p]),
    "nl_thin_decide_host": (_int, [_p, _i64, _p]),
}
ALL_SYMBOLS = sorted(list(_PROTOS) + list(_PLAIN))


class NellieHipError(RuntimeError):
    def __init__(self, code, msg):
        super().__init__(msg)
        self.code = code


class LibraryUnavailable(RuntimeError):
    """libnellie_hip.so is not built or cannot be loaded (as opposed to an error the loaded library reports)."""


# ... 273 lines not shown
    ndim = int(ndim) if shape is None else len(shape)
    if ndim not in (2, 3):
        raise ValueError(f"{what} are 2-D or 3-D, got {got}")
    if shape is not None:
        shape = tuple(int(s) for s in shape)
    sp = np.ascontiguousarray(spacing, dtype=np.float64)
    if sp.size != ndim:
        raise ValueError(f"spacing needs {ndim} values")
    return ndim, shape, (None if shape is None else (1,) * (3 - ndim) + shape), sp


def _frame_array(a, shape, what, owner, dtype=None, dtype_error=TypeError):
    a = np.asarray(a)
    if a.shape != shape:
        raise ValueError(f"{what} shape {a.shape} does not match the {owner}'s {shape}")
    if dtype is None and a.dtype not in DTYPE_CODES:
        raise dtype_error(f"unsupported {what} dtype {a.dtype}")
    if dtype is not None and a.dtype != dtype and np.dtype(dtype).kind in "iu":
        _refuse_lossy_cast(a, np.dtype(dtype), what)
    return np.ascontiguousarray(a, dtype=dtype)


def _refuse_lossy_cast(a, dtype, what):
    if a.size == 0 or a.dtype.kind == "b":
        return
    if a.dtype.kind not in "iuf":
        raise TypeError(f"{what} of dtype {a.dtype} cannot be converted to {dtype}")
    if a.dtype.kind == "f":
        bad = ~np.isfinite(a)
        if not bad.any():
            bad = a != np.trunc(a)
        if bad.any():
            raise ValueError(f"{what} holds {a[bad].flat[0].item()!r}, which {dtype} cannot hold: refusing a cast that changes values")
    info = np.iinfo(dtype)
    for v in (a.min(), a.max()):
        if not info.min <= int(v) <= info.max:
            raise ValueError(f"{what} holds {int(v)}, outside {dtype}'s range [{info.min}, {info.max}]: refusing a cast that changes values")


def _kernel_ms(handle, name) -> float:
    ms = _f32(0)
    handle._call(name, C.byref(ms))
    return float(ms.value)


class Context(_Handle):

    _destroy, _noun = "nl_ctx_destroy", "context"

    def __init__(self, shape, device=0, gz0=0, gnz=None, own=None):
        nz, ny, nx = (int(s) for s in shape)
        self.shape = (nz, ny, nx)
        self.gz0 = int(gz0)
        self.gnz = int(gnz) if gnz is not None else nz
        self.own = (0, nz) if own is None else (int(own[0]), int(own[1]))
        self.device = int(device)
        self._create("nl_ctx_create", self.device, nz, ny, nx, self.gz0, self.gnz, self.own[0], self.own[1])

    def sync(self):
        self._call("nl_sync")

    def filter_load(self, frame: np.ndarray, z0=0, z1=None):
        z1 = self.shape[0] if z1 is None else z1
        a = np.ascontiguousarray(frame)
        if a.dtype not in DTYPE_CODES:
            a = a.astype(np.float32)
        assert a.shape == (z1 - z0, self.shape[1], self.shape[2]), (a.shape, self.shape, z0, z1)
        self._call("nl_filter_load", _ptr(a), DTYPE_CODES[a.dtype], z0, z1)

    def input_load(self, frame: np.ndarray, z0=0, z1=None):
        z1 = self.shape[0] if z1 is None else z1
        a = np.ascontiguousarray(frame)
        if a.dtype not in DTYPE_CODES:
            a = a.astype(np.float32)
        assert a.shape == (z1 - z0, self.shape[1], self.shape[2]), (a.shape, self.shape, z0, z1)
        self._call("nl_input_load", _ptr(a), DTYPE_CODES[a.dtype], z0, z1)

    def filter_begin(self):
        self._call("nl_filter_begin")

    def gauss_commit(self):
        self._call("nl_gauss_commit")

    def gauss_step(self, wz, wy, wx, z0=0, z1=None, ahead=False):
        z1 = self.shape[0] if z1 is None else z1
        args = []
        keep = []
        for w in (wz, wy, wx):
            if w is None:
                args += [None, 0]
            else:
                w = np.ascontiguousarray(w, dtype=np.float64)
                keep.append(w)
                args += [_ptr(w), (len(w) - 1) // 2]
        self._call("nl_gauss_step_ahead" if ahead else "nl_gauss_step", *args, z0, z1)

    def sample_gather(self, field, strides):
        sz, sy, sx = (int(s) for s in strides)
        n = _i64(0)
        self._call("nl_sample_gather", field, sz, sy, sx, None, 0, C.byref(n))
        out = np.empty(int(n.value), dtype=np.float32)
        if out.size:
            self._call("nl_sample_gather", field, sz, sy, sx, _ptr(out), out.size, C.byref(n))
        return out

    def sample_gather_positive(self, field, strides):
        sz, sy, sx = (int(s) for s in strides)
        n = _i64(0)
        self._call("nl_sample_gather", field, sz, sy, sx, None, 0, C.byref(n))
        out = np.empty(int(n.value), dtype=np.float32)
        if out.size:
            self._call("nl_sample_gather_positive", field, sz, sy, sx, _ptr(out), out.size, C.byref(n))
        return out[:int(n.value)]

    def sample_gather_positive_begin(self, field, strides):
        sz, sy, sx = (int(s) for s in strides)
        n = _i64(0)
        self._call("nl_sample_gather_positive_begin", field, sz, sy, sx, C.byref(n))
        self._gp_cap = int(n.value)

    def sample_gather_positive_end(self):
        out = np.empty(self._gp_cap, dtype=np.float32)
        n = _i64(0)
        self._call("nl_sample_gather_positive_end", _ptr(out), out.size, C.byref(n))
        return out[:int(n.value)]

    def sample_minmax(self, field, strides):
        sz, sy, sx = (int(s) for s in strides)
        mn, mx, n = _f32(0), _f32(0), _i64(0)
        self._call("nl_sample_minmax", field, sz, sy, sx, C.byref(mn), C.byref(mx), C.byref(n))
        return np.float32(mn.value), np.float32(mx.value), int(n.value)

    def sample_hist(self, field, strides, edges: np.ndarray):
        sz, sy, sx = (int(s) for s in strides)
        e = np.ascontiguousarray(edges, dtype=np.float32)
        counts = np.zeros(e.size - 1, dtype=np.int64)
        self._call("nl_sample_hist", field, sz, sy, sx, _ptr(e), e.size - 1, _ptr(counts))
        return counts

    def sample_range_hist(self, field, strides, nbins=256):
        mn, mx, n, valid = _f32(0), _f32(0), _i64(0), _int(0)
        counts = np.zeros(nbins, np.int64)
        edges = np.zeros(nbins + 1, np.float32)
        sz, sy, sx = (int(s) for s in strides)
        self._call("nl_sample_range_hist", int(field), sz, sy, sx, int(nbins), C.byref(mn), C.byref(mx), C.byref(n),
                   _ptr(counts), _ptr(edges), C.byref(valid))
        return np.float32(mn.value), np.float32(mx.value), int(n.value), counts, edges, int(valid.value)

    def sample_range_hist2(self, field_a, field_b, strides, nbins=256):
        mn, mx, n, valid = np.zeros(2, np.float32), np.zeros(2, np.float32), np.zeros(2, np.int64), np.zeros(2, np.int32)
        counts = np.zeros((2, nbins), np.int64)
        edges = np.zeros((2, nbins + 1), np.float32)
        sz, sy, sx = (int(s) for s in strides)
        self._call("nl_sample_range_hist2", int(field_a), int(field_b), sz, sy, sx, int(nbins), _ptr(mn), _ptr(mx), _ptr(n),
                   _ptr(counts), _ptr(edges), _ptr(valid))
        return tuple((np.float32(mn[k]), np.float32(mx[k]), int(n[k]), counts[k], edges[k], int(valid[k])) for k in range(2))

    def hessian_stats(self, spacing):
        sp = (_f64 * 3)(*[float(s) for s in spacing])
        ma, mf, inf = _f32(0), _f32(0), _int(0)
        self._call("nl_hessian_stats", sp, C.byref(ma), C.byref(mf), C.byref(inf))
        return np.float32(ma.value), np.float32(mf.value), bool(inf.value)

    def set_frob_norm(self, max_abs, max_finite):
        self._call("nl_set_frob_norm", float(max_abs), float(max_finite))

    def vesselness_step(self, gamma_sq, alpha_sq, beta_sq, thr, want_count=True, z0=-1, z1=-1):
        n = _i64(0)
        use = 0 if thr is None else 1
        self._call("nl_vesselness_step", float(np.float32(gamma_sq)), float(np.float32(alpha_sq)),
                   float(np.float32(beta_sq)), use, float(np.float32(0.0 if thr is None else thr)),
                   int(z0), int(z1), C.byref(n) if want_count else None)
        return int(n.value)

    def mask_volume_fused(self, thr) -> int:
        n = _i64(0)
        self._call("nl_mask_volume_fused", float(np.float32(thr)), C.byref(n))
        return int(n.value)
# ... 149 lines not shown
        self._call("nl_thin_info", counts, ms)
        return dict(zip(self.THIN_COUNTS, (int(v) for v in counts))), float(ms[0])

    def network_clean_seed(self):
        a, b = _i64(0), _i64(0)
        self._call("nl_network_clean_seed", C.byref(a), C.byref(b))
        return int(a.value), int(b.value)

    def network_classes(self):
        a, b = _i64(0), _i64(0)
        self._call("nl_network_classes", C.byref(a), C.byref(b))
        return int(a.value), int(b.value)

    def network_relabel_load(self, labels, branch):
        labels = self._network_frame(labels, "labels", np.int32)
        branch = self._network_frame(branch, "branch labels", np.int32, labels.shape)
        self._network_shape = labels.shape
        n = _i64(0)
        self._call("nl_network_relabel_load", _ptr(labels), _ptr(branch), labels.ndim, C.byref(n))
        return int(n.value)

    def network_relabel(self, spacing, scratch_voxels=None):
        sp = np.ascontiguousarray(spacing, dtype=np.float64)
        if sp.size != len(self._network_shape):
            raise ValueError(f"spacing needs {len(self._network_shape)} values")
        a, b, k = _i64(0), _i64(0), _i64(0)
        self._call("nl_network_relabel", sp.ctypes.data_as(C.POINTER(_f64)), int(scratch_voxels or 0), C.byref(a), C.byref(b), C.byref(k))
        return int(a.value), int(b.value), int(k.value)

    def network_fetch(self, branch=True, pixel_class=True, relabelled=True):
        shape = self._network_shape
        s = np.empty(shape, np.int32) if branch else None
        p = np.empty(shape, np.uint8) if pixel_class else None
        r = np.empty(shape, np.uint32) if relabelled else None
        self._call("nl_network_fetch", _opt(s), _opt(p), _opt(r))
        return s, p, r

    def network_kernel_ms(self):
        ms = (_f32 * 4)()
        self._call("nl_network_kernel_ms", ms)
        return dict(zip(("clean", "seed", "classes", "relabel"), (float(v) for v in ms)))

    def set_ndim(self, ndim: int):
        self._call("nl_set_ndim", int(ndim))

    def log2d_step(self, wy2, wy0, wx2, wx0, s2, first, use_mask=True):
        arrs = [np.ascontiguousarray(w, dtype=np.float64) for w in (wy2, wy0, wx2, wx0)]
        r = (arrs[0].size - 1) // 2
        assert all(a.size == 2 * r + 1 for a in arrs)
        self._call("nl_log2d_step", *[a.ctypes.data_as(C.POINTER(_f64)) for a in arrs], r, float(np.float32(s2)),
                   1 if first else 0, 1 if use_mask else 0)

    def log2d_finish(self) -> int:
        n = _i64(0)
        self._call("nl_log2d_finish", C.byref(n))
        return int(n.value)

    def one_pass_available(self) -> bool:
        return bool(self.info("vesselness_one_pass"))

    def chain_available(self) -> bool:
        return bool(self.info("chain_available"))

    def set_spacing(self, spacing):
        sp = (_f64 * 3)(*[float(s) for s in spacing])
        self._call("nl_set_spacing", sp)

    def vesselness_spec(self, spacing, fsq_lo, fsq_hi, z0=-1, z1=-1):
        sp = (_f64 * 3)(*[float(s) for s in spacing])
        ma, mf, inf, ovf = _f32(0), _f32(0), _int(0), _int(0)
        self._call("nl_vesselness_spec", sp, float(np.float32(fsq_lo)), float(np.float32(fsq_hi)), int(z0), int(z1),
                   C.byref(ma), C.byref(mf), C.byref(inf), C.byref(ovf))
        return np.float32(ma.value), np.float32(mf.value), bool(inf.value), bool(ovf.value)

    def chain_begin(self, n_scales):
        self._call("nl_chain_begin", int(n_scales))
        self._chain_n = int(n_scales)

    def chain_scale(self, spacing, strides, alpha_sq, beta_sq, division, margin, test_scale=1.0, z0=-1, z1=-1):
        sp = (_f64 * 3)(*[float(s) for s in spacing])
        sz, sy, sx = (int(s) for s in strides)
        self._call("nl_chain_scale", sp, sz, sy, sx, float(alpha_sq), float(beta_sq), float(division), float(margin), float(test_scale),
                   int(z0), int(z1))

    def chain_flush(self):
        self._call("nl_chain_flush")

    def chain_finish(self):
        n = self._chain_n
        flags = np.zeros(n, np.int32)
        gamma, max_abs, thr = np.zeros(n), np.zeros(n), np.zeros(n)
        counts = np.zeros(n, np.int64)
        self._call("nl_chain_finish", _ptr(flags), _ptr(gamma), _ptr(max_abs), _ptr(thr), _ptr(counts))
        return flags, gamma, max_abs, thr, counts

    def chain_log(self, k, which):
        counts, edges = np.zeros(256, np.int64), np.zeros(257, np.float32)
        rng, sc = np.zeros(2, np.float32), np.zeros(8)
        self._call("nl_chain_log", int(k), int(which), _ptr(counts), _ptr(edges), _ptr(rng), _ptr(sc))
        return counts, edges, rng, dict(zip(("fsq_lo", "fsq_hi", "gamma_sq", "fsq_min", "thr_cmp", "max_frob", "tri", "otsu"), sc))

    def vesselness_resolve(self, gamma_sq, alpha_sq, beta_sq, thr) -> bool:
        hit = _int(0)
        use = 0 if thr is None else 1
        self._call("nl_vesselness_resolve", float(np.float32(gamma_sq)), float(np.float32(alpha_sq)),
                   float(np.float32(beta_sq)), use, float(np.float32(0.0 if thr is None else thr)),
                   C.byref(hit), None)
        return bool(hit.value)

    def vesselness_count(self) -> int:
        n = _i64(0)
        self._call("nl_vesselness_count", C.byref(n))
        return int(n.value)

    def filter_finish(self, z0=-1, z1=-1) -> int:
        n = _i64(0)
        self._call("nl_filter_finish", int(z0), int(z1), C.byref(n))
        return int(n.value)

    def remove_edges(self, margin=15) -> int:
        n = _i64(0)
        self._call("nl_remove_edges", int(margin), C.byref(n))
        return int(n.value)

    def planes_get(self, field, z0, z1):
        out = np.empty((z1 - z0, self.shape[1], self.shape[2]), dtype=np.float32)
        self._call("nl_planes_get", int(field), int(z0), int(z1), _ptr(out))
        return out

    def planes_put(self, field, z0, z1, planes):
        a = np.ascontiguousarray(planes, dtype=np.float32)
        assert a.shape == (z1 - z0, self.shape[1], self.shape[2])
        self._call("nl_planes_put", int(field), int(z0), int(z1), _ptr(a))

    def comm_init(self, world, rank, uid: bytes):
        assert len(uid) == 128
        self._call("nl_comm_init", int(world), int(rank), uid)

    def halo_exchange(self, field, depth):
        self._call("nl_halo_exchange", int(field), int(depth))

    def halo_exchange_at(self, field, offset, depth, run_async=False):
        self._call("nl_halo_exchange_at", int(field), int(offset), int(depth), 1 if run_async else 0)

    def comm_init2(self, world, rank, uid: bytes):
        self._call("nl_comm_init2", int(world), int(rank), uid)

    def allreduce(self, arr: np.ndarray, op: str):
        a = np.ascontiguousarray(arr)
        assert a.dtype in (np.int64, np.float32)
        self._call("nl_allreduce", _ptr(a), a.size, 0 if a.dtype == np.int64 else 1, {"sum": 0, "min": 1, "max": 2}[op])
        return a

    def mask_volume(self, thr):
        self._call("nl_mask_volume", float(np.float32(thr)))

    def filter_store(self, z0=0, z1=None, out=None):
        z1 = self.shape[0] if z1 is None else z1
        if out is None:
            out = np.empty((z1 - z0, self.shape[1], self.shape[2]), dtype=np.float32)
        assert out.dtype == np.float32 and out.flags.c_contiguous
        self._call("nl_filter_store", _ptr(out), z0, z1)
        return out

    def gauss_store(self, z0=0, z1=None):
        z1 = self.shape[0] if z1 is None else z1
# ... 525 lines not shown
```

### nellie_amd/pipeline.py

```python
from __future__ import annotations

from dataclasses import dataclass, field
from typing import Optional

import os

import numpy as np

from nellie_amd import hipnative
from nellie_amd.hipnative import FIELD_FRANGI, FIELD_FROB, FIELD_GAUSS, FIELD_VESSELNESS
from nellie_amd.utils.gpu_functions import (histogram_edges, min_triangle_otsu, otsu_threshold,
                                            triangle_threshold)

_EPS32 = float(np.finfo(np.float32).eps)
_TRUNCATE = 3.0


def z_ratio_of(dim_res) -> float:
    z_res = dim_res.get("Z") or dim_res.get("X") or 1.0
    x_res = dim_res.get("X") or 1.0
    return float(z_res) / float(x_res)


def spacing_of(dim_res):
# ... 89 lines not shown
        return [sigma_min], max_r
    step = max(0.2, rng / max(num_sigma, 1))
    sig = list(np.arange(sigma_min, sigma_max, step))
    return (sig if len(sig) else [sigma_min]), max_r


_DELTAS_CACHE = {}


def cascade_deltas(sigmas, z_ratio):
    key = (tuple(float(s) for s in sigmas), float(z_ratio))
    got = _DELTAS_CACHE.get(key)
    if got is None:
        got = _cascade_deltas(sigmas, z_ratio)
        if len(_DELTAS_CACHE) < 256:
            _DELTAS_CACHE[key] = got
    return list(got)


def _cascade_deltas(sigmas, z_ratio):
    out = []
    prev = 0.0
    for sigma in sigmas:
        vp = (float(prev) / z_ratio, float(prev), float(prev))
        vc = (float(sigma) / z_ratio, float(sigma), float(sigma))
        delta = []
        for sp, sc in zip(vp, vc):
            diff = max(0.0, float(sc) ** 2 - float(sp) ** 2)
            delta.append(np.sqrt(diff))
        out.append(tuple(delta))
        prev = sigma
    return out


def min_area_pixels_of(dim_res, min_radius_um=0.25, no_z=False):
    x_res = dim_res.get("X") or 1.0
    y_res = dim_res.get("Y") or x_res
    r = max(float(min_radius_um), float(x_res))
    if no_z:
        area_px = (np.pi * (r ** 2)) / (float(x_res) * float(y_res))
        return max(1, int(np.ceil(area_px)))
    z_res = dim_res.get("Z") or x_res
    volume_um3 = (4.0 / 3.0) * np.pi * (r ** 3)
    volume_px = volume_um3 / (float(x_res) * float(y_res) * float(z_res))
    return max(1, int(np.ceil(volume_px)))


@dataclass
class FilterParams:
    dim_res: dict
    min_radius_um: float = 0.25
    max_radius_um: float = 1.0
    alpha_sq: float = 0.5
    beta_sq: float = 0.5
    frob_thresh: Optional[float] = None
    frob_thresh_division: object = 2
    max_threshold_samples: int = int(1e6)
    sigmas: Optional[list] = None

    def resolved_sigmas(self):
        if self.sigmas is not None:
            return list(self.sigmas)
        return default_sigmas(self.dim_res, self.min_radius_um, self.max_radius_um)


@dataclass
class ScaleTrace:
    sigma: float
    gamma: float
    max_abs: float
    frob_thr: Optional[float]
    mask_count: int
    skipped: bool
    one_pass: bool = False


@dataclass
class FrameTrace:
    scales: list = field(default_factory=list)
    n_positive: int = 0
    percentile_thr: Optional[float] = None
    label_thr: Optional[float] = None
    n_labels: int = 0


class FramePipeline:

    def __init__(self, shape, device: int = 0, ctx=None):
        self.shape = tuple(int(s) for s in shape)
        self.two_d = len(self.shape) == 2
        if self.two_d:
            self.shape = (1,) + self.shape
        if len(self.shape) != 3:
            raise ValueError("FramePipeline takes a (Z, Y, X) or a (Y, X) shape")
        self.ctx = ctx if ctx is not None else hipnative.Context(self.shape, device=device)
        if self.two_d:
            self.ctx.set_ndim(2)
        self.trace = FrameTrace()
        self.one_pass = bool(getattr(self.ctx, "one_pass_available", lambda: False)()) and not self.two_d
        self.one_pass_margin = 1e-3
        self._chain_hist = hasattr(self.ctx, "sample_range_hist") and os.environ.get("NELLIE_CHAIN_HIST", "1") != "0"
        self._pair_hist = hasattr(self.ctx, "sample_range_hist2") and os.environ.get("NELLIE_PAIR_HIST", "1") != "0"
        self.check_device_edges = os.environ.get("NELLIE_CHECK_EDGES", "0") == "1"
        self._one_pass_test_scale = 1.0
        try:
            self._yx_max_r = int(self.ctx.info("gauss_yx_max_r"))
        except (KeyError, AttributeError):
            self._yx_max_r = 0

    def _step_fits_ahead(self, ws) -> bool:
        wz, wy, wx = ws
        n = 0 if wz is None else 1
        if wy is not None and wx is not None and len(wy) == len(wx) and 1 <= (len(wy) - 1) // 2 <= min(self._yx_max_r, self.shape[1]):
            n += 1
        else:
            n += (wy is not None) + (wx is not None)
        return n <= 2

    def close(self):
        self.ctx.close()

    def _strides(self, max_samples):
        if self.two_d:
            return (1,) + tuple(sample_strides(self.shape[1:], max_samples))
        return sample_strides(self.shape, max_samples)

    def _positive_lattice_samples(self, fld, strides):
        f = getattr(self.ctx, "sample_gather_positive", None)
        if f is not None:
            return self._gather(f(fld, strides))
        sample = self._gather(self.ctx.sample_gather(fld, strides))
        return sample[sample > 0]

    def _positive_flat_samples(self, fld, offset, step):
        f = getattr(self.ctx, "flat_sample_gather_positive", None)
        if f is not None:
            return self._gather(f(fld, offset, step))
        sample = self._gather(self.ctx.flat_sample_gather(fld, offset, step))
        return sample[sample > 0]

    def _as_frame(self, a):
        a = np.asarray(a)
        return a[None] if (self.two_d and a.ndim == 2) else a

    def _after_load(self, p):
        pass

    def _gauss_range(self, rz):
        return 0, self.shape[0]

    def _after_cascade_step(self, k):
        pass

    def _vess_range(self):
        return -1, -1

    def _reduce_minmax(self, mn, mx, npos):
        return mn, mx, npos

    def _reduce_counts(self, counts):
        return counts

    def _reduce_stats(self, max_abs, max_fsq, any_inf, overflow=0, fused_call=False):
        return max_abs, max_fsq, any_inf, overflow

    def _reduce_sum(self, n):
# ... 133 lines not shown
                pair = ctx.sample_range_hist2(FIELD_GAUSS, FIELD_FROB, strides, 256)
            gamma = self._threshold_from_field(FIELD_GAUSS, strides, pre=None if pair is None else pair[0])
            if gamma is None or gamma <= 0:
                gamma = _EPS32
            gamma_sq = 2.0 * (float(gamma) ** 2)
            spec = False
            stats = None
            if want_bracket:
                if pair is None:
                    ctx.set_spacing(spacing)
                bracket = self._fsq_bracket(strides, float(p.frob_thresh_division), None if pair is None else pair[1])
                if bracket is not None:
                    settle()
                    vz0, vz1 = self._vess_range()
                    ma, mf, inf_, ovf = ctx.vesselness_spec(spacing, bracket[0], bracket[1], z0=vz0, z1=vz1)
                    stats = self._reduce_stats(ma, mf, inf_, ovf, fused_call=True)
                    spec = not stats[2] and not stats[3]
                    if stats[2]:
                        stats = None
            if stats is None:
                stats = self._reduce_stats(*ctx.hessian_stats(spacing))
            max_abs32, max_fsq32, any_inf = stats[:3]
            max_abs = float(max_abs32)
            if max_abs <= 0:
                max_abs = 1.0
            with np.errstate(over="ignore", invalid="ignore", divide="ignore"):
                max_frob = np.sqrt(np.float32(max_fsq32)) / np.float32(max_abs)
            ctx.set_frob_norm(max_abs, float(max_frob) if any_inf else 0.0)
            thr = None
            if not mask:
                thr_cmp, nonempty = np.float32(-np.inf), True
            elif not p.frob_thresh_division:
                thr_cmp = None
                nonempty = bool(max_frob > 0)
            else:
                if p.frob_thresh is None:
                    t = self._threshold_from_field(FIELD_FROB, strides, self._normalised_range(spec, max_abs))
                    thr = 0.0 if t is None else t
                else:
                    thr = float(p.frob_thresh)
                thr_cmp = np.float32(thr / p.frob_thresh_division)
                nonempty = bool(max_frob > thr_cmp)
            count = 0
            hit = False
            if nonempty:
                if spec:
                    hit = ctx.vesselness_resolve(gamma_sq, alpha_sq, beta_sq, thr_cmp)
                if not hit:
                    settle()
                    vz0, vz1 = self._vess_range()
                    count = self._reduce_sum(ctx.vesselness_step(gamma_sq, alpha_sq, beta_sq, thr_cmp, z0=vz0, z1=vz1))
            self.trace.scales.append(ScaleTrace(float(sigma), float(gamma), max_abs, thr, count, not nonempty, hit))
            if hit:
                settle()
                pending = self.trace.scales[-1]
        settle()
        if not mask and not self.two_d:
            if self._reduce_sum(int(ctx.info("nan_hessian"))):
                raise np.linalg.LinAlgError("Eigenvalues did not converge")
        return self._finish_frame(finish, p, mask)

    _device_chain = os.environ.get("NELLIE_DEVICE_CHAIN", "1") == "1"
    chain_fallbacks = 0

    def _chain_usable(self, p: FilterParams, mask: bool) -> bool:
        return bool(self._device_chain and (self.one_pass or self.two_d) and mask and p.frob_thresh is None and p.frob_thresh_division
                    and hasattr(self.ctx, "chain_begin") and getattr(self.ctx, "chain_available", lambda: True)()
                    and self._chain_reductions_on_device())

    def _chain_reductions_on_device(self) -> bool:
        return True

    def _scales_on_the_device(self, p: FilterParams, max_samples: int) -> bool:
        ctx = self.ctx
        zr = z_ratio_of(p.dim_res)
        spacing = spacing_of(p.dim_res)
        sigmas = p.resolved_sigmas()
        if not 1 <= len(sigmas) <= 16:
            return False
        strides = self._strides(max_samples)
        deltas = list(cascade_deltas(sigmas, zr))
        if self.two_d:
            deltas = [(0.0, d[1], d[2]) for d in deltas]
        ctx.chain_begin(len(sigmas))
        run_ahead = self._chain_ahead(int(np.prod(self.shape))) and not self.two_d
        ahead = False
        margin = 1.0 if self.two_d else self.one_pass_margin

        def cascade_step(k, on_side):
            delta = deltas[k]
            if not any(s > 0 for s in delta):
                return False
            ws = [gaussian_weights(d) for d in delta]
            if on_side and not self._step_fits_ahead(ws):
                return False
            z0, z1 = self._gauss_range(0 if ws[0] is None else (len(ws[0]) - 1) // 2)
            ctx.gauss_step(*ws, z0=z0, z1=z1, **({"ahead": True} if on_side else {}))
            return True

        for k in range(len(sigmas)):
            if ahead:
                ctx.gauss_commit()
            else:
                cascade_step(k, False)
            self._after_cascade_step(k)
            ahead = run_ahead and k + 1 < len(sigmas) and cascade_step(k + 1, True)
            vz0, vz1 = self._vess_range()
            ctx.chain_scale(spacing, strides, float(p.alpha_sq), float(p.beta_sq), float(p.frob_thresh_division), margin,
                            self._one_pass_test_scale, z0=vz0, z1=vz1)
        dev_tail = self._tail_field is not None and self._device_tail_usable()
        tail = not dev_tail and self._tail_ok and self._tail_field is not None and hasattr(ctx, "sample_gather_positive_begin")
        self._tail_samples = None
        self._tail_dev_pending = False
        if dev_tail:
            ctx.chain_flush()
            ctx.tail_enqueue(strides, 1.0)
        elif tail:
            ctx.chain_flush()
            ctx.sample_gather_positive_begin(self._tail_field, strides)
        flags, gamma, max_abs, thr, counts = ctx.chain_finish()
        samples = ctx.sample_gather_positive_end() if tail else None
        self.last_chain_flags = [int(f) for f in flags]
        if not self._all_ranks_agree(not flags.any()):
            if dev_tail:
                ctx.tail_finish(commit=False)
            return False
        self._tail_samples = samples
        self._tail_dev_pending = dev_tail
        if self.check_device_edges:
            for k in range(len(sigmas)):
                for which in range(3):
                    _, edges, rng, _ = ctx.chain_log(k, which)
                    assert np.array_equal(edges, histogram_edges(rng[0], rng[1], 256)), "device-built histogram edges differ from numpy's"
        for k, sigma in enumerate(sigmas):
            self.trace.scales.append(ScaleTrace(float(sigma), float(gamma[k]), float(max_abs[k]), float(thr[k]),
                                                self._reduce_mask_count(int(counts[k])), False, not self.two_d))
        return True

    def _all_ranks_agree(self, ok: bool) -> bool:
        return ok

    _chain_ahead_env = None

    def _chain_ahead(self, n_voxels: int) -> bool:
        env = self._chain_ahead_env if self._chain_ahead_env is not None else os.environ.get("NELLIE_CHAIN_AHEAD")
        if env is not None:
            return env == "1"
        return n_voxels < (1 << 26)

    def _finish_frame(self, finish: bool, p: FilterParams, mask: bool):
        ctx = self.ctx
        sigmas = p.resolved_sigmas()
        self._settle_mask_counts()
        if not finish:
            return None
        vz0, vz1 = self._vess_range()
        self.trace.n_positive = self._reduce_sum(ctx.filter_finish(vz0, vz1))
        if self.two_d:
            for i, s in enumerate(sigmas):
                w2, w0 = gaussian_derivative_weights(s, 2), gaussian_derivative_weights(s, 0)
                ctx.log2d_step(w2, w0, w2, w0, np.float32(float(s) ** 2), first=(i == 0), use_mask=mask)
            self.trace.n_positive = ctx.log2d_finish()
        return self.trace.n_positive

    def _load(self, frame):
        self.ctx.filter_load(self._as_frame(frame))

    def mask_volume(self, p: FilterParams):
        strides = self._strides(int(p.max_threshold_samples))
        if self._device_percentile_usable():
            rec = self.ctx.mask_volume_dev(strides, 1.0)
            if rec["n_samples"] == 0:
                return None
            self._check_device_percentile(rec)
            self.trace.percentile_thr = float(rec["thr"])
            return rec["thr"]
        positive = self._positive_lattice_samples(FIELD_FRANGI, strides)
        if positive.size == 0:
            return None
        thr = percentile_of_samples(positive, 1)
        self.ctx.mask_volume(thr)
        self.trace.percentile_thr = float(thr)
        return thr

    _tail_ok = True
    _tail_field = None
    _tail_samples = None
    _tail_dev_pending = False
    _device_tail = os.environ.get("NELLIE_DEVICE_TAIL", "1") == "1"

    def _device_percentile_usable(self) -> bool:
        global _FAST_PERCENTILE
# ... 199 lines not shown
```

### nellie_amd/sharded.py

```python
from __future__ import annotations

import os

import numpy as np

from nellie_amd import hipnative
from nellie_amd.hipnative import FIELD_FRANGI, FIELD_GAUSS
from nellie_amd.pipeline import (FilterParams, FramePipeline, cascade_deltas, gaussian_weights, z_ratio_of)


def slab_range(gnz: int, world: int, rank: int):
    base, rem = divmod(int(gnz), int(world))
    o0 = rank * base + min(rank, rem)
    return o0, o0 + base + (1 if rank < rem else 0)


def halo_depth(p: FilterParams) -> int:
    sig = p.resolved_sigmas()
    rz = 0
    for delta in cascade_deltas(sig, z_ratio_of(p.dim_res)):
        w = gaussian_weights(delta[0])
        rz += 0 if w is None else (len(w) - 1) // 2
    return rz + 4

# ... 65 lines not shown
        allr = np.concatenate([np.asarray(x, np.int64) for x in rt]) if rt else np.zeros(0, np.int64)
        allv = np.concatenate([np.asarray(x, np.int64) for x in vt]) if vt else np.zeros(0, np.int64)
        u, first, inv = np.unique(allr, return_index=True, return_inverse=True)
        cuts = np.cumsum([0] + [len(x) for x in rt])
        ids.append([n + inv[cuts[k]:cuts[k + 1]] for k in range(4)])
        ranks.append(np.full(u.size, r, np.int64)); roots.append(u); vals.append(allv[first])
        n += u.size
    ea, eb = [], []
    for r in range(len(tables) - 1):
        for mine, theirs in ((2, 0), (3, 1)):
            a, b = ids[r][mine], ids[r + 1][theirs]
            if a.size != b.size:
                raise RuntimeError(f"slab tables of ranks {r} and {r + 1} disagree ({a.size} vs {b.size} runs): the ghost bit planes are stale")
            ea.append(a); eb.append(b)
    j = _Joined()
    j.rank = np.concatenate(ranks) if ranks else np.zeros(0, np.int64)
    j.root = np.concatenate(roots).astype(np.int32) if roots else np.zeros(0, np.int32)
    j.val = np.concatenate(vals) if vals else np.zeros(0, np.int64)
    if n == 0:
        j.comp, j.ncomp = np.zeros(0, np.int64), 0
        return j
    ea = np.concatenate(ea) if ea else np.zeros(0, np.int64)
    eb = np.concatenate(eb) if eb else np.zeros(0, np.int64)
    j.ncomp, j.comp = _components(n, ea, eb)
    return j


def _components(n, ea, eb):
    lab = np.arange(n, dtype=np.int64)
    if ea.size:
        while True:
            m = np.minimum(lab[ea], lab[eb])
            new = lab.copy()
            np.minimum.at(new, ea, m)
            np.minimum.at(new, eb, m)
            new = new[new]
            if np.array_equal(new, lab):
                break
            lab = new
    u, comp = np.unique(lab, return_inverse=True)
    return int(u.size), comp.astype(np.int64)


class RcclComm:

    def __init__(self, ctx, world, rank, uid: bytes, host_gather=None, uid2: bytes = None):
        self.world, self.rank = world, rank
        self.ctx = ctx
        ctx.comm_init(world, rank, uid)
        self.has_side_channel = uid2 is not None
        if uid2 is not None:
            ctx.comm_init2(world, rank, uid2)
        self.fused = os.environ.get("NELLIE_FUSE_REDUCE", "1") == "1"
        if self.fused:
            ctx.comm_fuse(True)

    def exchange_halo(self, ctx, field, depth, offset=0, run_async=False):
        ctx.halo_exchange_at(field, offset, depth, run_async and self.has_side_channel)

    def exchange_bits(self, ctx, which):
        ctx.slab_bits_exchange(which)

    def allreduce(self, arr, op):
        return self.ctx.allreduce(arr, op)

    def positive_samples_world(self, ctx, field, mode, a, b, c, block_items):
        return ctx.positive_samples_world(field, mode, a, b, c, block_items, self.world)

    def slab_phase_gather(self, ctx, phase):
        return ctx.slab_phase(phase, gather_world=self.world)

    def allgather_list(self, arr):
        return self.ctx.allgather_var(np.ascontiguousarray(arr), self.world)

    def allgather(self, arr):
        return np.concatenate(self.allgather_list(arr))

    def allgather_mask_bits(self, ctx, slab_plane0):
        ctx.label_bits_allgather(slab_plane0)


class ShardedFramePipeline(FramePipeline):
    _tail_ok = False

    def __init__(self, gshape, rank, world, comm_factory, params: FilterParams, device: int = 0, ctx_factory=None, halo=None,
                 halo_mode=None):
        import os
        self.rank, self.world = int(rank), int(world)
        self.halo_mode = halo_mode or os.environ.get("NELLIE_HALO", "steps")
        if self.halo_mode not in ("steps", "fat"):
            raise ValueError(f"halo_mode must be 'steps' or 'fat', not {self.halo_mode!r}")
        self._rz = step_radii(params)
        need = halo_depth_steps(params) if self.halo_mode == "steps" else halo_depth(params)
        self.halo = need if halo is None else int(halo)
        self._filter_ok = self.halo >= need
        lshape, gz0, own_lo, own_hi = slab_geometry(gshape, world, rank, self.halo)
        self.lshape, self.gz0, self.own = lshape, gz0, (own_lo, own_hi)
        make = ctx_factory or (lambda shp, dev, g0, gn, own: hipnative.Context(shp, device=dev, gz0=g0, gnz=gn, own=own))
        ctx = make(lshape, device, gz0, int(gshape[0]), (own_lo, own_hi))
        super().__init__(gshape, device=device, ctx=ctx)
        self.comm = comm_factory(ctx)
        self._gauss_ahead = hasattr(ctx, "gauss_commit") and os.environ.get("NELLIE_GAUSS_AHEAD", "1") == "1"
        self._fused_reduce = bool(getattr(self.comm, "fused", False))
        self._chain_hist = self._fused_reduce
        self.params = params
        self._valid = (0, lshape[0])
        self._raw_ghosts_loaded = False
        self._fused_epilogue = hasattr(ctx, "mask_volume_fused") and hasattr(ctx, "sample_gather_positive")

    def raw_ghost_needed(self):
        if self.halo_mode == "fat":
            return self.own[0], self.lshape[0] - self.own[1]
        lo, hi = self.own
        d = 4 + self._rz[0]
        return min(d, lo), min(d, self.lshape[0] - hi)

    def _place(self, frame):
        lo, hi = self.own
        n = np.shape(frame)[0]
        g_lo, g_hi = self.raw_ghost_needed()
        if n == hi - lo:
            self._raw_ghosts_loaded = (g_lo == 0 and g_hi == 0)
            return lo, hi
        if n == hi - lo + g_lo + g_hi:
            self._raw_ghosts_loaded = True
            return lo - g_lo, hi + g_hi
        raise ValueError(f"a frame of {n} planes is neither the {hi - lo} owned planes nor those plus the {g_lo} + {g_hi} raw ghost planes")

    def _load(self, frame):
        z0, z1 = self._place(frame)
        self.ctx.filter_load(np.asarray(frame), z0=z0, z1=z1)

    def load_input(self, frame):
        z0, z1 = self._place(frame)
        self.ctx.input_load(np.asarray(frame), z0=z0, z1=z1)

    def _after_load(self, p):
        if not self._filter_ok:
            raise ValueError(f"this slab holds {self.halo} ghost planes, the {self.halo_mode!r} exchange scheme of Filter needs more")
        lo, hi = self.own
        nzl = self.lshape[0]
        have = self._raw_ghosts_loaded
        if self.halo_mode == "fat":
            depth = max(lo, nzl - hi)
            if depth and not have:
                self.comm.exchange_halo(self.ctx, FIELD_GAUSS, depth)
            self._valid = (0, nzl)
        elif self.world > 1 and not have:
            self.comm.exchange_halo(self.ctx, FIELD_GAUSS, 4 + self._rz[0], 0, False)


    def _gauss_range(self, rz):
        nzl = self.lshape[0]
        if self.halo_mode == "steps":
            lo, hi = self.own
            return max(lo - 4, 0), min(hi + 4, nzl)
        v0, v1 = self._valid
        z0 = v0 if self.gz0 + v0 == 0 else v0 + rz
        z1 = v1 if self.gz0 + v1 == self.shape[0] else v1 - rz
        z0 = max(z0, 0)
        z1 = min(z1, nzl)
        self._valid = (z0, z1)
        return z0, z1

    def _after_cascade_step(self, k):
        if self.halo_mode == "steps" and self.world > 1 and k + 1 < len(self._rz) and self._rz[k + 1] > 0:
# ... 173 lines not shown
```

Measured before the change: 28790 Mvoxel/s.

## Walk Frangi scales out of sigma order using predicted mask fractions

Splits each chain scale into a sample phase (first-round histogram and threshold, plus a predicted above-threshold fraction over the sample lattice) and a separate walk/resolve phase. Up to three Gaussian volumes and parked fsq caches let a scale's walk wait up to two cascade steps, so scales can be walked in a chosen or auto order (lowest predicted fraction first). The point is to reorder scales so the max-accumulating vesselness resolve can skip more voxels or reuse cached work. It adds host syncs for the estimates, state bookkeeping, and only applies to single-context 3-D runs where every cascade step is fused.

```diff
diff --git a/include/nellie_amd.h b/include/nellie_amd.h
--- a/include/nellie_amd.h
+++ b/include/nellie_amd.h
@@ -110,6 +110,15 @@
 int nl_chain_flush(nl_ctx *ctx, char *err, size_t errlen);
 int nl_chain_finish(nl_ctx *ctx, int *flags, double *gamma, double *max_abs, double *thr, int64_t *mask_count, char *err, size_t errlen);
 int nl_chain_log(nl_ctx *ctx, int k, int which, int64_t *counts, float *edges, float *range, double *scalars, char *err, size_t errlen);
+
+int nl_gauss_step_fused(nl_ctx *ctx, const double *wz, int rz, const double *wy, int ry, const double *wx, int rx, int *fused,
+                        char *err, size_t errlen);
+int nl_chain_begin_unordered(nl_ctx *ctx, int n_scales, char *err, size_t errlen);
+int nl_chain_sample(nl_ctx *ctx, int k, const double spacing[3], int64_t sz, int64_t sy, int64_t sx, double division, double margin,
+                    double test_scale, char *err, size_t errlen);
+int nl_chain_estimates(nl_ctx *ctx, float *frac, int n, char *err, size_t errlen);
+int nl_chain_walk(nl_ctx *ctx, int k, const double spacing[3], int64_t sz, int64_t sy, int64_t sx, double alpha_sq, double beta_sq,
+                  double division, int64_t z0, int64_t z1, char *err, size_t errlen);
 
 int nl_vesselness_resolve(nl_ctx *ctx, float gamma_sq, float alpha_sq, float beta_sq, int use_thr, float thr,
                           int *hit, int64_t *mask_count, char *err, size_t errlen);
diff --git a/nellie_amd/csrc/chain.inc b/nellie_amd/csrc/chain.inc
--- a/nellie_amd/csrc/chain.inc
+++ b/nellie_amd/csrc/chain.inc
@@ -26,6 +26,8 @@
     int status_gauss, status_raw, status_exact;
     double tri[3], otsu[3];
     ChainHist h_gauss, h_raw, h_exact;
+    float pred_frac;
+    int pad_;
 };
 
 __device__ inline int wave_argmax_f64(const double *a, int n) {
@@ -147,7 +149,7 @@
 __device__ inline bool dev_finite_f(float x) { return fabsf(x) <= 3.402823466e38f; }
 
 __global__ void __launch_bounds__(64)
-chain_thr1_kernel(ChainScale *cs, double division, double margin, double test_scale) {
+chain_thr1_kernel(ChainScale *cs, double division, double margin, double test_scale, double n_lattice) {
     __shared__ double scratch[6 * NL_CHAIN_BINS];
     int flags = 0;
     if (blockIdx.x == 0) {
@@ -188,7 +190,17 @@
         if (!(dev_finite_f(l) && dev_finite_f(u) && u > 0.0f) || !(l <= u)) flags |= NL_CF_BRACKET;
         else { lo = l; hi = u; }
     }
+    float pred = -1.0f;
+    if (!flags && n_lattice > 0.0) {
+        unsigned long long part = 0;
+        for (int i = threadIdx.x; i < NL_CHAIN_BINS; i += 64) {
+            const float centre = (h.edges[i] + h.edges[i + 1]) / 2.0f;
+            if (centre * centre >= lo) part += h.counts[i];
+        }
+        pred = (float)((double)wave_sum_u64(part) / n_lattice);
+    }
     if (threadIdx.x == 0) {
+        cs->pred_frac = pred;
         cs->tri[1] = tri1; cs->otsu[1] = otsu1; cs->status_raw = st1;
         cs->raw_mn = raw_mn; cs->raw_mx = raw_mx;
         cs->fsq_lo = lo; cs->fsq_hi = hi;
diff --git a/nellie_amd/csrc/nellie_hip.hip b/nellie_amd/csrc/nellie_hip.hip
--- a/nellie_amd/csrc/nellie_hip.hip
+++ b/nellie_amd/csrc/nellie_hip.hip
@@ -172,6 +172,8 @@
     if (c->d_blk) hipFree(c->d_blk);
     for (int k = 0; k < 4; ++k) if (c->d_2d[k]) hipFree(c->d_2d[k]);
     if (c->d_fsq_cache) hipFree(c->d_fsq_cache);
+    for (auto &pk : c->fsq_park) if (pk.p) hipFree(pk.p);
+    if (c->h_chain_est) hipHostFree(c->h_chain_est);
     if (c->d_vq) hipFree(c->d_vq);
     if (c->mk_scratch) hipFree(c->mk_scratch);
     if (c->mk_act) hipFree(c->mk_act);
@@ -328,7 +330,7 @@
     NL_JOIN_SIDE(c);
     if (!host || z0 < 0 || z1 > c->nzl || z0 >= z1) return nl_fail(err, errlen, NL_EINVAL, "bad plane range [%lld,%lld)", (i64)z0, (i64)z1);
     c->i_gauss = 0; c->i_vmax = 3; c->i_labels = -1; c->frangi_ready = 0;
-    c->pz_on = 0; c->prezero_used = 0;
+    c->pz_on = 0; c->prezero_used = 0; c->chain_reorder = 0;
     c->gauss_ext = nullptr;
     if (c->ahead_pending) NL_HIP(hipStreamWaitEvent(c->stream, c->ev_ahead, 0));
     c->ahead_pending = 0;
@@ -363,7 +365,7 @@
     NL_JOIN_SIDE(c);
     if (!c->d_input) return nl_fail(err, errlen, NL_ESTATE, "nl_filter_begin before nl_input_load");
     c->i_gauss = 0; c->i_vmax = 3; c->i_labels = -1; c->frangi_ready = 0;
-    c->pz_on = 0; c->prezero_used = 0;
+    c->pz_on = 0; c->prezero_used = 0; c->chain_reorder = 0;
     c->mask_slots_used = 0;
     c->gauss_ext = nullptr;
     if (c->ahead_pending) NL_HIP(hipStreamWaitEvent(c->stream, c->ev_ahead, 0));
@@ -402,6 +404,19 @@
     return (wz ? 1 : 0) + (gauss_can_yx(c, wy, ry, wx, rx) ? 1 : (wy ? 1 : 0) + (wx ? 1 : 0));
 }
 
+static bool gauss_takes_zyx(const nl_ctx *c, const double *wz, int rz, const double *wy, int ry, const double *wx, int rx) {
+    const char *e_fz = getenv("NELLIE_GAUSS_FUSED");
+    const bool fused_zyx = e_fz ? atoi(e_fz) != 0 : c->n >= ((i64)1 << 26);
+    return fused_zyx && wz && gauss_can_yx(c, wy, ry, wx, rx) && gyx_tiled() && gl_zyx_ok(c, rz, ry, c->f[(c->i_gauss + 1) % 3]) &&
+           memcmp(wy, wx, (size_t)(2 * ry + 1) * sizeof(double)) == 0;
+}
+extern "C" int nl_gauss_step_fused(nl_ctx *c, const double *wz, int rz, const double *wy, int ry, const double *wx, int rx, int *fused,
+                                   char *err, size_t errlen) {
+    if (!c || !fused) return nl_fail(err, errlen, NL_EINVAL, "ctx or fused is NULL");
+    *fused = gauss_takes_zyx(c, wz, rz, wy, ry, wx, rx) ? 1 : 0;
+    return NL_OK;
+}
+
 extern "C" int nl_gauss_step(nl_ctx *c, const double *wz, int rz, const double *wy, int ry, const double *wx, int rx,
                              int64_t z0, int64_t z1, char *err, size_t errlen) {
     NL_ENTER(c);
@@ -420,15 +435,20 @@
     int rc;
     const bool can_yx = gauss_can_yx(c, wy, ry, wx, rx);
     bool fused_yx = false;
-    const char *e_fz = getenv("NELLIE_GAUSS_FUSED");
-    const bool fused_zyx = e_fz ? atoi(e_fz) != 0 : c->n >= ((i64)1 << 26);
-    if (fused_zyx && wz && can_yx && gyx_tiled() && gl_zyx_ok(c, rz, ry, c->f[(src + 1) % 3]) &&
-        memcmp(wy, wx, (size_t)(2 * ry + 1) * sizeof(double)) == 0) {
+    const bool reorder = c->chain_reorder && c->chain_n > 0;
+    int dst_zyx = (src + 1) % 3;
+    if (reorder) {
+        if (c->vol_scale[dst_zyx] >= 0) dst_zyx = (src + 2) % 3;
+        if (c->vol_scale[dst_zyx] >= 0 || c->stream == c->side || !gauss_takes_zyx(c, wz, rz, wy, ry, wx, rx))
+            return nl_fail(err, errlen, NL_ESTATE, c->vol_scale[dst_zyx] >= 0 ? "no free Gaussian volume: three scales wait for their walk"
+                                                                                : "a chain out of sigma order takes fused cascade steps only");
+    }
+    if (gauss_takes_zyx(c, wz, rz, wy, ry, wx, rx)) {
         GaussW gy;
         if ((rc = fill_gw(gw, wz, rz, err, errlen)) || (rc = fill_gw(gy, wy, ry, err, errlen))) return rc;
         if ((z0 - rz < 0 && c->gz0 > 0) || (z1 - 1 + rz >= c->nzl && c->gz0 + c->nzl < c->gnz))
             return nl_fail(err, errlen, NL_EINVAL, "Z pass of radius %d on planes [%lld,%lld) reaches outside the local slab", rz, (i64)z0, (i64)z1);
-        const int dst = (src + 1) % 3;
+        const int dst = dst_zyx;
         char scope[32];
         snprintf(scope, sizeof scope, "gauss_zyx<%d,%d>", rz, ry);
         ProfScope ps(c, scope);
@@ -436,8 +456,11 @@
         if (zero_in_passing < 0) { const char *e = getenv("NELLIE_ZERO_IN_GAUSS"); zero_in_passing = (e && !atoi(e)) ? 0 : 1; }
         const bool zero = zero_in_passing && c->mask_slots_used == 0 && c->vmax_zero_hi == 0 && c->stream != c->side;
         const bool ahead = c->stream == c->side;
-        const bool prezero = !zero && c->pz_on && c->chain_n > 0 && c->chain_k == c->chain_n - (ahead ? 2 : 1) && z0 == 0 && z1 == c->nzl;
-        float *third = c->f[(src + 2) % 3];
+        const int i_third = 3 - src - dst;
+        const bool last = reorder ? (c->chain_steps == c->chain_n - 1 && c->vol_scale[i_third] < 0)
+                                  : c->chain_k == c->chain_n - (ahead ? 2 : 1);
+        const bool prezero = !zero && c->pz_on && c->chain_n > 0 && last && z0 == 0 && z1 == c->nzl;
+        float *third = c->f[i_third];
         (void)gl_zyx(c, rz, ry, srcp, c->f[dst], v, z0, z1, gauss_ws_of(gw), gauss_ws_of(gy), zero ? c->f[c->i_vmax] : (prezero ? third : nullptr));
         if (zero) { c->vmax_zero_lo = z0; c->vmax_zero_hi = z1; }
         NL_CHECK_LAUNCH();
@@ -488,6 +511,7 @@
     c->i_gauss = src;
     c->fsq_cache_valid = 0;
     if (srcp != c->gauss_ext) c->gauss_ext = nullptr;
+    if (reorder) ++c->chain_steps;
     return NL_OK;
 }
 
@@ -897,10 +921,16 @@
     NL_CHECK_LAUNCH();
     c->chain_n = n_scales; c->chain_k = 0; c->chain_copy_pending = 0;
     c->def_resolve = 0;
+    c->chain_reorder = 0; c->chain_steps = 0; c->chain_walked = 0;
+    for (int v = 0; v < 3; ++v) { c->vol_scale[v] = -1; c->fsq_park[v].valid = 0; }
     const char *e_pz = getenv("NELLIE_PREZERO");
     c->pz_on = (e_pz ? atoi(e_pz) != 0 : NL_PREZERO_DEFAULT) && !c->two_d && !c->comm && c->own_lo == 0 && c->own_hi == c->nzl && c->nzl == c->gnz;
     return NL_OK;
 }
+
+static int chain_first_round(nl_ctx *c, ChainScale *cs, i64 sz, i64 sy, i64 sx, double division, double margin, double test_scale, char *err, size_t errlen);
+static int chain_walk_resolve(nl_ctx *c, ChainScale *cs, const double spacing[3], i64 sz, i64 sy, i64 sx, double alpha_sq, double beta_sq, double division,
+                              int64_t z0, int64_t z1, char *err, size_t errlen);
 
 extern "C" int nl_chain_scale(nl_ctx *c, const double spacing[3], int64_t sz, int64_t sy, int64_t sx, double alpha_sq, double beta_sq,
                               double division, double margin, double test_scale, int64_t z0, int64_t z1, char *err, size_t errlen) {
@@ -916,7 +946,7 @@
     c->frob_max_abs = 1.0f; c->frob_max_finite = 0.0f;
     if (c->two_d) {
         if ((rc = sample_first_round(c, NL_FIELD_GAUSS, NL_FIELD_FROB, sz, sy, sx, NL_CHAIN_BINS, (char *)&cs->h_gauss, (char *)&cs->h_raw, nullptr, nullptr, true, err, errlen))) return rc;
-        chain_thr1_kernel<<<2, 64, 0, c->stream>>>(cs, division, margin, test_scale);
+        chain_thr1_kernel<<<2, 64, 0, c->stream>>>(cs, division, margin, test_scale, 0.0);
         {
             ProfScope ps(c, "hessian_stats");
             hessian2d_stats_kernel<<<grid2d_rows(c->nx, c->ny), 256, 0, c->stream>>>(gauss_cur(c), geom(c), hessp(c), cs->stats);
@@ -946,9 +976,23 @@
         NL_CHECK_LAUNCH();
         return NL_OK;
     }
+    if ((rc = chain_first_round(c, cs, sz, sy, sx, division, margin, test_scale, err, errlen))) return rc;
+    return chain_walk_resolve(c, cs, spacing, sz, sy, sx, alpha_sq, beta_sq, division, z0, z1, err, errlen);
+}
+
+static int chain_first_round(nl_ctx *c, ChainScale *cs, i64 sz, i64 sy, i64 sx, double division, double margin, double test_scale, char *err, size_t errlen) {
+    int rc;
     if ((rc = sample_first_round(c, NL_FIELD_GAUSS, NL_FIELD_FROB, sz, sy, sx, NL_CHAIN_BINS, (char *)&cs->h_gauss, (char *)&cs->h_raw, nullptr, nullptr, true, err, errlen))) return rc;
-    chain_thr1_kernel<<<2, 64, 0, c->stream>>>(cs, division, margin, test_scale);
-    NL_CHECK_LAUNCH();
+    const i64 g_lo = c->gz0 + c->own_lo, g_hi = c->gz0 + c->own_hi;
+    const i64 cz = (g_hi + sz - 1) / sz - (g_lo + sz - 1) / sz;
+    const double n_lattice = (double)((cz > 0 ? cz : 0) * ((c->ny + sy - 1) / sy) * ((c->nx + sx - 1) / sx));
+    chain_thr1_kernel<<<2, 64, 0, c->stream>>>(cs, division, margin, test_scale, n_lattice);
+    NL_CHECK_LAUNCH();
+    return NL_OK;
+}
+static int chain_walk_resolve(nl_ctx *c, ChainScale *cs, const double spacing[3], i64 sz, i64 sy, i64 sx, double alpha_sq, double beta_sq, double division,
+                              int64_t z0, int64_t z1, char *err, size_t errlen) {
+    int rc;
     if ((rc = spec_enqueue(c, spacing, 0.0f, 0.0f, z0, z1, cs->stats, &cs->cnt_walk, &cs->fsq_lo, err, errlen))) return rc;
     const bool defer = resolve_defer_ok(c) && c->fsq_cache_valid;
     hipStream_t st = c->stream;
@@ -969,6 +1013,77 @@
     return resolve_enqueue(c, vp, &cs->cnt_resolve, (const float *)cs, err, errlen);
 }
 
+extern "C" int nl_chain_begin_unordered(nl_ctx *c, int n_scales, char *err, size_t errlen) {
+    int rc = nl_chain_begin(c, n_scales, err, errlen);
+    if (rc) return rc;
+    if (c->two_d || c->comm) { c->chain_n = 0; return nl_fail(err, errlen, NL_ESTATE, "scales out of sigma order: whole 3-D volumes on one context only"); }
+    c->chain_reorder = 1;
+    return NL_OK;
+}
+
+static void fsq_swap_parked(nl_ctx *c, int v) {
+    nl_ctx::FsqPark &pk = c->fsq_park[v];
+    std::swap(pk.p, c->d_fsq_cache); std::swap(pk.cap, c->fsq_cache_cap); std::swap(pk.valid, c->fsq_cache_valid);
+    for (int i = 0; i < 3; ++i) std::swap(pk.key[i], c->fsq_cache_key[i]);
+}
+
+extern "C" int nl_chain_sample(nl_ctx *c, int k, const double spacing[3], int64_t sz, int64_t sy, int64_t sx, double division, double margin,
+                               double test_scale, char *err, size_t errlen) {
+    NL_ENTER_KEEP_PZ(c);
+    if (!c->d_chain || !c->chain_reorder || c->chain_n < 1) return nl_fail(err, errlen, NL_ESTATE, "nl_chain_sample outside nl_chain_begin_unordered .. nl_chain_finish");
+    if (k != c->chain_k || k >= c->chain_n) return nl_fail(err, errlen, NL_ESTATE, "nl_chain_sample(%d): scale %d is the next in sigma order", k, c->chain_k);
+    if (c->chain_steps != k + 1 || c->gauss_ext) return nl_fail(err, errlen, NL_ESTATE, "nl_chain_sample(%d) without a cascade step of its own", k);
+    if (!(division != 0.0)) return nl_fail(err, errlen, NL_EINVAL, "the chain needs a non-zero threshold division");
+    int rc;
+    if ((rc = set_spacing(c, spacing, err, errlen))) return rc;
+    if ((rc = resolve_deferred_launch(c, true, err, errlen))) return rc;
+    c->chain_par[k][0] = division; c->chain_par[k][1] = margin; c->chain_par[k][2] = test_scale;
+    c->frob_max_abs = 1.0f; c->frob_max_finite = 0.0f;
+    if ((rc = chain_first_round(c, (ChainScale *)c->d_chain + k, sz, sy, sx, division, margin, test_scale, err, errlen))) return rc;
+    const int v = c->i_gauss;
+    fsq_swap_parked(c, v);
+    c->fsq_cache_valid = 0;
+    c->vol_scale[v] = k; c->chain_vol[k] = v;
+    ++c->chain_k;
+    return NL_OK;
+}
+
+extern "C" int nl_chain_estimates(nl_ctx *c, float *frac, int n, char *err, size_t errlen) {
+    NL_ENTER_KEEP_PZ(c);
+    if (!c->d_chain || !c->chain_reorder || c->chain_n < 1) return nl_fail(err, errlen, NL_ESTATE, "nl_chain_estimates outside nl_chain_begin_unordered .. nl_chain_finish");
+    if (!frac || n < 0 || n > NL_CHAIN_MAX_SCALES) return nl_fail(err, errlen, NL_EINVAL, "bad arguments");
+    if (!c->h_chain_est) NL_HIP(hipHostMalloc((void **)&c->h_chain_est, sizeof(float) * NL_CHAIN_MAX_SCALES, hipHostMallocDefault));
+    const int have = c->chain_k < n ? c->chain_k : n;
+    for (int k = 0; k < have; ++k)
+        NL_HIP(hipMemcpyAsync(c->h_chain_est + k, &((const ChainScale *)c->d_chain)[k].pred_frac, sizeof(float), hipMemcpyDeviceToHost, c->stream));
+    if (have) NL_HIP(hipStreamSynchronize(c->stream));
+    for (int k = 0; k < n; ++k) frac[k] = k < have ? c->h_chain_est[k] : -1.0f;
+    return NL_OK;
+}
+
+extern "C" int nl_chain_walk(nl_ctx *c, int k, const double spacing[3], int64_t sz, int64_t sy, int64_t sx, double alpha_sq, double beta_sq,
+                             double division, int64_t z0, int64_t z1, char *err, size_t errlen) {
+    NL_ENTER_KEEP_PZ(c);
+    if (!c->d_chain || !c->chain_reorder || c->chain_n < 1) return nl_fail(err, errlen, NL_ESTATE, "nl_chain_walk outside nl_chain_begin_unordered .. nl_chain_finish");
+    if (k < 0 || k >= c->chain_k || ((c->chain_walked >> k) & 1u)) return nl_fail(err, errlen, NL_ESTATE, "nl_chain_walk(%d): the scale is not pending", k);
+    const int v = c->chain_vol[k];
+    if (c->vol_scale[v] != k) return nl_fail(err, errlen, NL_ESTATE, "nl_chain_walk(%d): its Gaussian is gone", k);
+    int rc;
+    if ((rc = set_spacing(c, spacing, err, errlen))) return rc;
+    if ((rc = resolve_deferred_launch(c, false, err, errlen))) return rc;
+    fsq_swap_parked(c, v);
+    c->frob_max_abs = 1.0f; c->frob_max_finite = 0.0f;
+    const int newest = c->i_gauss;
+    c->i_gauss = v;
+    rc = chain_walk_resolve(c, (ChainScale *)c->d_chain + k, spacing, sz, sy, sx, alpha_sq, beta_sq, division, z0, z1, err, errlen);
+    c->i_gauss = newest;
+    c->fsq_cache_valid = 0;
+    if (rc) return rc;
+    c->vol_scale[v] = -1;
+    c->chain_walked |= 1u << k;
+    return NL_OK;
+}
+
 extern "C" int nl_chain_flush(nl_ctx *c, char *err, size_t errlen) {
     NL_ENTER_KEEP_PZ(c);
     if (!c->d_chain || c->chain_k < 1) return nl_fail(err, errlen, NL_ESTATE, "nl_chain_flush without scales");
@@ -984,6 +1099,7 @@
     NL_ENTER_KEEP_PZ(c);
     if (!c->d_chain || c->chain_k < 1) return nl_fail(err, errlen, NL_ESTATE, "nl_chain_finish without scales");
     const int n = c->chain_k;
+    if (c->chain_reorder && c->chain_walked != (1u << n) - 1u) return nl_fail(err, errlen, NL_ESTATE, "nl_chain_finish while a sampled scale waits for its walk");
     if (!c->chain_copy_pending) { int rcd = resolve_deferred_launch(c, false, err, errlen); if (rcd) return rcd; }
     if (c->chain_copy_pending) {
         NL_HIP(hipEventSynchronize(c->ev_chain));
@@ -1002,7 +1118,7 @@
         if (thr) thr[k] = (double)h[k].thr;
         if (mask_count) mask_count[k] = (int64_t)(h[k].cnt_walk + h[k].cnt_resolve);
     }
-    c->chain_n = 0; c->pz_on = 0;
+    c->chain_n = 0; c->pz_on = 0; c->chain_reorder = 0;
     return NL_OK;
 }
 
diff --git a/nellie_amd/csrc/nl_common.h b/nellie_amd/csrc/nl_common.h
--- a/nellie_amd/csrc/nl_common.h
+++ b/nellie_amd/csrc/nl_common.h
@@ -137,6 +137,13 @@
     void *d_chain = nullptr, *h_chain = nullptr;
     int chain_n = 0, chain_k = 0;
     double chain_par[16][3] = {};
+    int chain_reorder = 0;
+    int chain_steps = 0;
+    unsigned chain_walked = 0;
+    int chain_vol[16] = {};
+    int vol_scale[3] = {-1, -1, -1};
+    struct FsqPark { float *p = nullptr; i64 cap = 0, key[3] = {0, 0, 0}; int valid = 0; } fsq_park[3];
+    float *h_chain_est = nullptr;
 
     void *comm = nullptr;
     int fuse_reduce = 0;
diff --git a/nellie_amd/hipnative.py b/nellie_amd/hipnative.py
--- a/nellie_amd/hipnative.py
+++ b/nellie_amd/hipnative.py
@@ -133,6 +133,11 @@
     "nl_chain_flush": [_p],
     "nl_chain_finish": [_p, _p, _p, _p, _p, _p],
     "nl_chain_log": [_p, _int, _int, _p, _p, _p, _p],
+    "nl_gauss_step_fused": [_p, _p, _int, _p, _int, _p, _int, C.POINTER(_int)],
+    "nl_chain_begin_unordered": [_p, _int],
+    "nl_chain_sample": [_p, _int, _p, _i64, _i64, _i64, _f64, _f64, _f64],
+    "nl_chain_estimates": [_p, _p, _int],
+    "nl_chain_walk": [_p, _int, _p, _i64, _i64, _i64, _f64, _f64, _f64, _i64, _i64],
     "nl_pinned_alloc": [C.POINTER(_p), _i64],
     "nl_host_register": [_p, _i64],
     "nl_input_load_async": [_p, _int, _p, _int],
@@ -572,18 +577,28 @@
     def gauss_commit(self):
         self._call("nl_gauss_commit")
 
-    def gauss_step(self, wz, wy, wx, z0=0, z1=None, ahead=False):
-        z1 = self.shape[0] if z1 is None else z1
-        args = []
-        keep = []
-        for w in (wz, wy, wx):
+    @staticmethod
+    def _weight_args(ws):
+        args, keep = [], []
+        for w in ws:
             if w is None:
                 args += [None, 0]
             else:
                 w = np.ascontiguousarray(w, dtype=np.float64)
                 keep.append(w)
                 args += [_ptr(w), (len(w) - 1) // 2]
+        return args, keep
+
+    def gauss_step(self, wz, wy, wx, z0=0, z1=None, ahead=False):
+        z1 = self.shape[0] if z1 is None else z1
+        args, keep = self._weight_args((wz, wy, wx))
         self._call("nl_gauss_step_ahead" if ahead else "nl_gauss_step", *args, z0, z1)
+
+    def gauss_step_fused(self, wz, wy, wx) -> bool:
+        args, keep = self._weight_args((wz, wy, wx))
+        fused = _int(0)
+        self._call("nl_gauss_step_fused", *args, C.byref(fused))
+        return bool(fused.value)
 
     def sample_gather(self, field, strides):
         sz, sy, sx = (int(s) for s in strides)
@@ -899,6 +914,25 @@
         sz, sy, sx = (int(s) for s in strides)
         self._call("nl_chain_scale", sp, sz, sy, sx, float(alpha_sq), float(beta_sq), float(division), float(margin), float(test_scale),
                    int(z0), int(z1))
+
+    def chain_begin_unordered(self, n_scales):
+        self._call("nl_chain_begin_unordered", int(n_scales))
+        self._chain_n = int(n_scales)
+
+    def chain_sample(self, k, spacing, strides, division, margin, test_scale=1.0):
+        sp = (_f64 * 3)(*[float(s) for s in spacing])
+        sz, sy, sx = (int(s) for s in strides)
+        self._call("nl_chain_sample", int(k), sp, sz, sy, sx, float(division), float(margin), float(test_scale))
+
+    def chain_estimates(self):
+        frac = np.full(self._chain_n, -1.0, np.float32)
+        self._call("nl_chain_estimates", _ptr(frac), int(frac.size))
+        return frac
+
+    def chain_walk(self, k, spacing, strides, alpha_sq, beta_sq, division, z0=-1, z1=-1):
+        sp = (_f64 * 3)(*[float(s) for s in spacing])
+        sz, sy, sx = (int(s) for s in strides)
+        self._call("nl_chain_walk", int(k), sp, sz, sy, sx, float(alpha_sq), float(beta_sq), float(division), int(z0), int(z1))
 
     def chain_flush(self):
         self._call("nl_chain_flush")
diff --git a/nellie_amd/pipeline.py b/nellie_amd/pipeline.py
--- a/nellie_amd/pipeline.py
+++ b/nellie_amd/pipeline.py
@@ -195,6 +195,34 @@
     percentile_thr: Optional[float] = None
     label_thr: Optional[float] = None
     n_labels: int = 0
+
+
+def run_scale_schedule(n, order, step, walk, choose):
+    pending, done, newest, pos = [], 0, None, 0
+    while pos < n:
+        busy = set(pending) | ({newest} if newest is not None else set())
+        can_step = done < n and len(busy) <= 2
+        want = order[pos] if order is not None else None
+        if can_step and done == n - 1 and not set(pending) <= {newest}:
+            can_step = want is not None and want not in pending
+        if can_step:
+            step(done)
+            pending.append(done)
+            newest = done
+            done += 1
+            continue
+        if want is None:
+            want = choose(list(pending), n - done)
+        if want not in pending:
+            return False
+        walk(want)
+        pending.remove(want)
+        pos += 1
+    return True
+
+
+def scale_order_fits(order) -> bool:
+    return run_scale_schedule(len(order), list(order), lambda k: None, lambda k: None, None)
 
 
 class FramePipeline:
@@ -494,7 +522,22 @@
         deltas = list(cascade_deltas(sigmas, zr))
         if self.two_d:
             deltas = [(0.0, d[1], d[2]) for d in deltas]
-        ctx.chain_begin(len(sigmas))
+        order = self._scale_order(deltas)
+        if order is None:
+            self._scales_in_sigma_order(p, spacing, strides, deltas)
+        else:
+            self._scales_out_of_order(p, spacing, strides, deltas, order)
+        return self._chain_epilogue(strides, sigmas)
+
+    _chain_test_scales = {}
+
+    def _chain_test_scale(self, k):
+        return self._chain_test_scales.get(k, self._one_pass_test_scale)
+
+    def _scales_in_sigma_order(self, p, spacing, strides, deltas):
+        ctx = self.ctx
+        n = len(deltas)
+        ctx.chain_begin(n)
         run_ahead = self._chain_ahead(int(np.prod(self.shape))) and not self.two_d
         ahead = False
         margin = 1.0 if self.two_d else self.one_pass_margin
@@ -510,16 +553,81 @@
             ctx.gauss_step(*ws, z0=z0, z1=z1, **({"ahead": True} if on_side else {}))
             return True
 
-        for k in range(len(sigmas)):
+        for k in range(n):
             if ahead:
                 ctx.gauss_commit()
             else:
                 cascade_step(k, False)
             self._after_cascade_step(k)
-            ahead = run_ahead and k + 1 < len(sigmas) and cascade_step(k + 1, True)
+            ahead = run_ahead and k + 1 < n and cascade_step(k + 1, True)
             vz0, vz1 = self._vess_range()
             ctx.chain_scale(spacing, strides, float(p.alpha_sq), float(p.beta_sq), float(p.frob_thresh_division), margin,
-                            self._one_pass_test_scale, z0=vz0, z1=vz1)
+                            self._chain_test_scale(k), z0=vz0, z1=vz1)
+
+    _scale_reorder_ok = True
+    last_scale_order = None
+    _all_steps_fused = {}
+
+    def _scale_order(self, deltas):
+        self.last_scale_order = None
+        env = os.environ.get("NELLIE_SCALE_ORDER", "auto").strip().lower() or "auto"
+        if env == "sigma" or not self._scale_reorder_ok or self.two_d or not hasattr(self.ctx, "chain_begin_unordered"):
+            return None
+        if self._chain_ahead(int(np.prod(self.shape))):
+            return None
+        key = (tuple(deltas), os.environ.get("NELLIE_GAUSS_FUSED"))
+        if key not in self._all_steps_fused:
+            self._all_steps_fused = {key: all(all(s > 0 for s in d) and self.ctx.gauss_step_fused(*[gaussian_weights(s) for s in d])
+                                              for d in deltas)}
+        if not self._all_steps_fused[key]:
+            return None
+        if env == "auto":
+            return "auto"
+        n = len(deltas)
+        try:
+            order = [int(t) - 1 for t in env.split(",")]
+        except ValueError:
+            raise ValueError(f"NELLIE_SCALE_ORDER={env!r}: expected auto, sigma or a permutation such as 3,2,1,4,5") from None
+        if sorted(order) != list(range(n)):
+            raise ValueError(f"NELLIE_SCALE_ORDER={env!r} is not a permutation of the frame's {n} scales (1..{n})")
+        if not scale_order_fits(order):
+            raise ValueError(f"NELLIE_SCALE_ORDER={env!r} cannot be scheduled inside three Gaussian volumes: a scale's walk can be "
+                             f"delayed by two cascade steps at most")
+        return order
+
+    def _scales_out_of_order(self, p, spacing, strides, deltas, order):
+        ctx = self.ctx
+        n = len(deltas)
+        ctx.chain_begin_unordered(n)
+        division = float(p.frob_thresh_division)
+        est = {}
+        walked = []
+
+        def step(k):
+            ws = [gaussian_weights(d) for d in deltas[k]]
+            z0, z1 = self._gauss_range((len(ws[0]) - 1) // 2)
+            ctx.gauss_step(*ws, z0=z0, z1=z1)
+            ctx.chain_sample(k, spacing, strides, division, self.one_pass_margin, self._chain_test_scale(k))
+
+        def walk(k):
+            vz0, vz1 = self._vess_range()
+            ctx.chain_walk(k, spacing, strides, float(p.alpha_sq), float(p.beta_sq), division, z0=vz0, z1=vz1)
+            walked.append(k)
+
+        def choose(pending, steps_left):
+            if len(pending) > 1 and steps_left and any(k not in est for k in pending):
+                for k, f in enumerate(ctx.chain_estimates()):
+                    if f >= 0:
+                        est[k] = float(f)
+            if any(k not in est for k in pending):
+                return min(pending)
+            return min(pending, key=lambda k: (est[k], k))
+
+        run_scale_schedule(n, None if order == "auto" else order, step, walk, choose)
+        self.last_scale_order = walked
+
+    def _chain_epilogue(self, strides, sigmas) -> bool:
+        ctx = self.ctx
         dev_tail = self._tail_field is not None and self._device_tail_usable()
         tail = not dev_tail and self._tail_ok and self._tail_field is not None and hasattr(ctx, "sample_gather_positive_begin")
         self._tail_samples = None
diff --git a/nellie_amd/sharded.py b/nellie_amd/sharded.py
--- a/nellie_amd/sharded.py
+++ b/nellie_amd/sharded.py
@@ -171,6 +171,7 @@
 
 class ShardedFramePipeline(FramePipeline):
     _tail_ok = False
+    _scale_reorder_ok = False
 
     def __init__(self, gshape, rank, world, comm_factory, params: FilterParams, device: int = 0, ctx_factory=None, halo=None,
                  halo_mode=None):
```

Result: faster. 30330 Mvoxel/s (median of 6 runs) (+5.3%).
